# hrdkjain/GenIcoNet

Hardware: AMD Instinct MI355X
Metric: meshes/sec training throughput, ico2ico I5 batch=36 (higher is better)
Workload: dtype f32; 1 GPU; ico2ico AE training, I5, batch 36 per GPU (BASELINE configs[1]); per_gpu_batch=36, global_batch=36, subdivisions=5, parallelism=dp1

## Files before the change

geniconet_amd/_lib.py:

```python
import ctypes
import os
import types

import numpy as np
import torch

_HERE = os.path.dirname(os.path.abspath(__file__))
LIB_PATH = os.environ.get('ICN_LIB_PATH') or os.path.join(_HERE, 'libicn.so')

OP_CONV_FWD, OP_CONV_BWD_DATA, OP_CONV_BWD_WEIGHT = 0, 1, 2
CORNER_MODES = {'zeros': 0, 'average': 1}
ABI_VERSION = 9
LAP_MODES = {'mean-v': 0, 'v-mean': 1, 'sum-kv': 2, 'kv-sum': 3}

_c_float_p = ctypes.c_void_p
_i32p = ctypes.POINTER(ctypes.c_int32)
_f32p = ctypes.POINTER(ctypes.c_float)
_intp = ctypes.POINTER(ctypes.c_int)

RC, COUNT, PLAIN = 'rc', 'count', 'plain'

SIGNATURES = {
    'icn_abi_version': (ctypes.c_int, [], PLAIN),
    'icn_last_error': (ctypes.c_char_p, [], PLAIN),
    'icn_prepare_conv': (ctypes.c_int, [ctypes.c_int] * 3, RC),
    'icn_prepare_upsample': (ctypes.c_int, [ctypes.c_int] * 2, RC),
    'icn_conv_workspace_bytes': (ctypes.c_size_t, [ctypes.c_int] * 6, PLAIN),
    'icn_conv_fwd': (ctypes.c_int, [_c_float_p] * 4 + [ctypes.c_int] * 6 + [ctypes.c_void_p, ctypes.c_size_t, ctypes.c_void_p], RC),
    'icn_conv_bwd_data': (ctypes.c_int, [_c_float_p] * 3 + [ctypes.c_int] * 6 + [ctypes.c_void_p, ctypes.c_size_t, ctypes.c_void_p], RC),
    'icn_conv_bwd_weight': (ctypes.c_int, [_c_float_p] * 4 + [ctypes.c_int] * 6 + [ctypes.c_void_p, ctypes.c_size_t, ctypes.c_void_p], RC),
    'icn_conv_pair_supported': (ctypes.c_int, [ctypes.c_int] * 6, PLAIN),
    'icn_conv_pair_workspace_bytes': (ctypes.c_size_t, [ctypes.c_int] * 7, PLAIN),
    'icn_conv_pair_fwd': (ctypes.c_int, [_c_float_p] * 7 + [ctypes.c_int] * 7 + [ctypes.c_void_p, ctypes.c_size_t, ctypes.c_void_p], RC),
    'icn_conv_pair_bwd_data': (ctypes.c_int, [_c_float_p] * 5 + [ctypes.c_int] * 7 + [ctypes.c_void_p, ctypes.c_size_t, ctypes.c_void_p], RC),
    'icn_conv_pair_bwd_weight': (ctypes.c_int, [_c_float_p] * 7 + [ctypes.c_int] * 7 + [ctypes.c_void_p, ctypes.c_size_t, ctypes.c_void_p], RC),
    'icn_upconv_supported': (ctypes.c_int, [ctypes.c_int] * 5, PLAIN),
    'icn_upconv_workspace_bytes': (ctypes.c_size_t, [ctypes.c_int] * 5, PLAIN),
    'icn_upconv_fwd': (ctypes.c_int, [_c_float_p] * 7 + [ctypes.c_int] * 6 + [ctypes.c_void_p, ctypes.c_size_t, ctypes.c_void_p], RC),
    'icn_upconv_bwd_supported': (ctypes.c_int, [ctypes.c_int] * 6, PLAIN),
    'icn_upconv_bwd_workspace_bytes': (ctypes.c_size_t, [ctypes.c_int] * 5, PLAIN),
    'icn_upconv_bwd': (ctypes.c_int, [_c_float_p] * 10 + [ctypes.c_int] * 6 + [ctypes.c_void_p, ctypes.c_size_t, ctypes.c_void_p], RC),
    'icn_upconv_bwd_streams': (ctypes.c_int, [_c_float_p] * 10 + [ctypes.c_int] * 6 + [ctypes.c_void_p, ctypes.c_size_t, ctypes.c_void_p, ctypes.c_void_p], RC),
    'icn_upsample_fwd': (ctypes.c_int, [_c_float_p] * 2 + [ctypes.c_int] * 4 + [ctypes.c_void_p], RC),
    'icn_upsample_bwd': (ctypes.c_int, [_c_float_p] * 2 + [ctypes.c_int] * 4 + [ctypes.c_void_p], RC),
    'icn_bn_workspace_floats': (ctypes.c_size_t, [ctypes.c_int] * 2, PLAIN),
    'icn_bn_stats2': (ctypes.c_int, [_c_float_p, _c_float_p, ctypes.c_int, ctypes.c_int] + ([ctypes.c_float] * 2 + [_c_float_p] * 3) * 2 + [_c_float_p, ctypes.c_void_p], RC),
    'icn_bn_stats': (ctypes.c_int, [_c_float_p, ctypes.c_int, ctypes.c_int, ctypes.c_float, ctypes.c_float] + [_c_float_p] * 4 + [ctypes.c_void_p], RC),
    'icn_bn_relu_fwd': (ctypes.c_int, [_c_float_p] * 9 + [ctypes.c_int] * 2 + [ctypes.c_void_p], RC),
    'icn_bn_relu_bwd': (ctypes.c_int, [_c_float_p] * 13 + [ctypes.c_int] * 2 + [_c_float_p] * 4 + [ctypes.c_void_p], RC),
    'icn_head_workspace_floats': (ctypes.c_size_t, [ctypes.c_int] * 2, PLAIN),
    'icn_head_fwd': (ctypes.c_int, [_c_float_p] * 4 + [ctypes.c_int] * 3 + [ctypes.c_void_p], RC),
    'icn_head_bwd': (ctypes.c_int, [_c_float_p] * 8 + [ctypes.c_int] * 3 + [ctypes.c_void_p], RC),
    'icn_p2p_loss_workspace_floats': (ctypes.c_size_t, [ctypes.c_int] * 2, PLAIN),
    'icn_p2p_loss_fwd': (ctypes.c_int, [_c_float_p] * 2 + [ctypes.c_int] * 2 + [ctypes.c_float] * 3 + [ctypes.c_int] + [_c_float_p] * 2 + [ctypes.c_void_p], RC),
    'icn_p2p_loss_bwd_workspace_floats': (ctypes.c_size_t, [ctypes.c_int] * 2, PLAIN),
    'icn_p2p_loss_bwd': (ctypes.c_int, [_c_float_p] * 3 + [ctypes.c_int] * 2 + [ctypes.c_float] * 3 + [ctypes.c_int] + [_c_float_p] * 2 + [ctypes.c_void_p], RC),
    'icn_mesh_reg_workspace_floats': (ctypes.c_size_t, [ctypes.c_int] * 2, PLAIN),
    'icn_mesh_reg_fwd': (ctypes.c_int, [_c_float_p] + [ctypes.c_int] * 2 + [ctypes.c_float] * 4 + [_c_float_p] * 2 + [ctypes.c_void_p], RC),
    'icn_mesh_reg_bwd_workspace_floats': (ctypes.c_size_t, [ctypes.c_int] * 2, PLAIN),
    'icn_mesh_reg_bwd': (ctypes.c_int, [_c_float_p] * 2 + [ctypes.c_int] * 2 + [ctypes.c_float] * 4 + [_c_float_p] * 2 + [ctypes.c_void_p], RC),
    'icn_kld_workspace_floats': (ctypes.c_size_t, [ctypes.c_size_t], PLAIN),
    'icn_kld_fwd': (ctypes.c_int, [_c_float_p] * 2 + [ctypes.c_size_t] + [_c_float_p] * 2 + [ctypes.c_void_p], RC),
    'icn_kld_bwd': (ctypes.c_int, [_c_float_p] * 3 + [ctypes.c_size_t] + [_c_float_p] * 2 + [ctypes.c_void_p], RC),
    'icn_reparam_fwd': (ctypes.c_int, [_c_float_p] * 3 + [ctypes.c_size_t] + [_c_float_p] + [ctypes.c_void_p], RC),
    'icn_reparam_bwd': (ctypes.c_int, [_c_float_p] * 3 + [ctypes.c_size_t] + [_c_float_p] * 2 + [ctypes.c_void_p], RC),
    'icn_adam_step': (ctypes.c_int, [ctypes.c_int] + [ctypes.c_void_p] * 7 + [ctypes.c_double] * 4 + [ctypes.c_void_p], RC),
    'icn_adam_step_dev': (ctypes.c_int, [ctypes.c_int] + [ctypes.c_void_p] * 6 + [ctypes.c_double] * 4 + [ctypes.c_void_p], RC),
    'icn_table_stream_k': (ctypes.c_long, [ctypes.c_int] * 4 + [_i32p, ctypes.c_size_t], COUNT),
    'icn_table_tile_lists': (ctypes.c_long, [ctypes.c_int] * 7 + [_i32p, ctypes.c_size_t], COUNT),
    'icn_set_debug_flags': (ctypes.c_int, [ctypes.c_int], PLAIN),
    'icn_device_status': (ctypes.c_int, [ctypes.c_int], COUNT),
    'icn_get_arith': (ctypes.c_int, [], COUNT),
    'icn_set_arith': (ctypes.c_int, [ctypes.c_int], COUNT),
    'icn_build_flags': (ctypes.c_uint, [], PLAIN),
    'icn_host_selfcheck': (ctypes.c_long, [ctypes.c_int] * 2, COUNT),
    'icn_debug_trace': (ctypes.c_int, [ctypes.c_void_p, ctypes.c_size_t], RC),
    'icn_point_to_mesh': (ctypes.c_int, [_c_float_p] * 3 + [ctypes.c_int] * 4 + [_c_float_p] * 3 + [ctypes.c_void_p], RC),
    'icn_point_to_mesh_bwd_workspace_bytes': (ctypes.c_size_t, [ctypes.c_int] * 4, PLAIN),
    'icn_point_to_mesh_grid_workspace_bytes': (ctypes.c_size_t, [ctypes.c_int] * 4, PLAIN),
    'icn_point_to_mesh_grid': (ctypes.c_int, [_c_float_p] * 3 + [ctypes.c_int] * 4 + [_c_float_p] * 3 + [ctypes.c_void_p, ctypes.c_size_t, ctypes.c_void_p], RC),
    'icn_point_to_mesh_bwd': (ctypes.c_int, [_c_float_p] * 6 + [ctypes.c_int] * 4 + [_c_float_p] * 2 + [ctypes.c_void_p, ctypes.c_size_t, ctypes.c_void_p], RC),
    'icn_mesh_sample_workspace_bytes': (ctypes.c_size_t, [ctypes.c_int] * 4, PLAIN),
    'icn_mesh_sample_fwd': (ctypes.c_int, [_c_float_p] * 3 + [ctypes.c_int] * 4 + [_c_float_p] * 3 + [ctypes.c_void_p, ctypes.c_size_t, ctypes.c_void_p], RC),
    'icn_mesh_sample_bwd_workspace_bytes': (ctypes.c_size_t, [ctypes.c_int] * 4, PLAIN),
    'icn_mesh_sample_bwd': (ctypes.c_int, [_c_float_p] * 4 + [ctypes.c_int] * 4 + [_c_float_p] + [ctypes.c_void_p, ctypes.c_size_t, ctypes.c_void_p], RC),
    'icn_table_conv_fwd': (ctypes.c_long, [ctypes.c_int] * 3 + [_i32p, ctypes.c_size_t], COUNT),
    'icn_table_wgrad7': (ctypes.c_long, [ctypes.c_int] * 3 + [_i32p, ctypes.c_size_t, ctypes.POINTER(ctypes.c_uint16), ctypes.c_size_t, _intp], COUNT),
    'icn_table_conv_bwd': (ctypes.c_long, [ctypes.c_int] * 3 + [_i32p, ctypes.c_size_t, _intp], COUNT),
    'icn_table_upsample': (ctypes.c_long, [ctypes.c_int] * 3 + [_i32p, _f32p, ctypes.c_size_t, _intp], COUNT),
    'icn_table_upsample_pairs': (ctypes.c_long, [ctypes.c_int, _i32p, ctypes.c_size_t], COUNT),
    'icn_table_faces': (ctypes.c_long, [ctypes.c_int, _i32p, ctypes.c_size_t], COUNT),
    'icn_table_vertex_stencils': (ctypes.c_long, [ctypes.c_int, _i32p, ctypes.c_size_t], COUNT),
    'icn_table_upconv_bwd': (ctypes.c_long, [ctypes.c_int] * 2 + [_i32p, _f32p, ctypes.c_size_t, _intp], COUNT),
    'icn_table_upconv': (ctypes.c_long, [ctypes.c_int, ctypes.c_int, _i32p, ctypes.c_size_t, _f32p, ctypes.c_size_t, _intp], COUNT),
}

EXTENSION_HEADERS = {
    'icn_ext.h': {
        'icn_face_normal_agree_bwd_workspace_bytes': (ctypes.c_size_t, [ctypes.c_int] * 4, PLAIN),
        'icn_face_normal_agree_fwd': (ctypes.c_int, ([_c_float_p] * 3 + [ctypes.c_int] * 2) * 2 + [ctypes.c_int] * 3 + [_c_float_p, ctypes.c_void_p], RC),
        'icn_face_normal_agree_bwd': (ctypes.c_int, ([_c_float_p] * 3 + [ctypes.c_int] * 2) * 2 + [ctypes.c_int] * 3 + [_c_float_p] * 3
                                      + [ctypes.c_void_p, ctypes.c_size_t, ctypes.c_void_p], RC),
    },
    'icn_measure.h': {
        'icn_mesh_measure_workspace_bytes': (ctypes.c_size_t, [ctypes.c_int] * 3, PLAIN),
        'icn_mesh_measure_fwd': (ctypes.c_int, [_c_float_p] * 2 + [ctypes.c_int] * 3 + [_c_float_p] * 2 + [ctypes.c_void_p, ctypes.c_size_t, ctypes.c_void_p], RC),
        'icn_mesh_measure_bwd': (ctypes.c_int, [_c_float_p] * 6 + [ctypes.c_int] * 3 + [_c_float_p, ctypes.c_void_p], RC),
    },
    'icn_curvature.h': {
        'icn_mesh_cotlap_fwd': (ctypes.c_int, [_c_float_p] * 4 + [ctypes.c_int] * 3 + [_c_float_p] * 2 + [ctypes.c_void_p], RC),
        'icn_mesh_cotlap_bwd': (ctypes.c_int, [_c_float_p] * 6 + [ctypes.c_int] * 3 + [_c_float_p, ctypes.c_void_p], RC),
        'icn_mesh_willmore_workspace_bytes': (ctypes.c_size_t, [ctypes.c_int] * 3, PLAIN),
        'icn_mesh_willmore_fwd': (ctypes.c_int, [_c_float_p] * 4 + [ctypes.c_int] * 3 + [_c_float_p] * 3 + [ctypes.c_void_p, ctypes.c_size_t, ctypes.c_void_p], RC),
        'icn_mesh_willmore_bwd': (ctypes.c_int, [_c_float_p] * 7 + [ctypes.c_int] * 3 + [_c_float_p, ctypes.c_void_p, ctypes.c_size_t, ctypes.c_void_p], RC),
    },
    'icn_gauss.h': {
        'icn_mesh_angle_defect_fwd': (ctypes.c_int, [_c_float_p] * 4 + [ctypes.c_int] * 3 + [_c_float_p, ctypes.c_void_p], RC),
        'icn_mesh_angle_defect_bwd': (ctypes.c_int, [_c_float_p] * 5 + [ctypes.c_int] * 3 + [_c_float_p, ctypes.c_void_p], RC),
    },
    'icn_isect.h': {
        'icn_mesh_self_intersect': (ctypes.c_int, [_c_float_p] * 2 + [ctypes.c_int] * 3 + [_c_float_p, ctypes.c_void_p], RC),
    },
    'icn_sdf.h': {
        'icn_point_to_mesh_sign': (ctypes.c_int, [_c_float_p] * 8 + [ctypes.c_int] * 4 + [_c_float_p, ctypes.c_void_p], RC),
    },
    'icn_voxel.h': {
        'icn_mesh_voxelize': (ctypes.c_int, [_c_float_p] * 2 + [ctypes.c_int] * 3 + [ctypes.c_double] * 4 + [ctypes.c_int] * 3
                              + [ctypes.c_void_p, ctypes.c_void_p], RC),
    },
    'icn_raycast.h': {
        'icn_mesh_raycast': (ctypes.c_int, [_c_float_p] * 4 + [ctypes.c_int] * 4 + [_c_float_p] * 3 + [ctypes.c_void_p], RC),
        'icn_mesh_raycast_bwd_workspace_bytes': (ctypes.c_size_t, [ctypes.c_int] * 3, PLAIN),
        'icn_mesh_raycast_bwd': (ctypes.c_int, [_c_float_p] * 6 + [ctypes.c_int] * 4 + [_c_float_p] * 3
                                 + [ctypes.c_void_p, ctypes.c_size_t, ctypes.c_void_p], RC),
    },
    'icn_nn.h': {
        'icn_nearest_points': (ctypes.c_int, [_c_float_p] * 2 + [ctypes.c_int] * 3 + [_c_float_p] * 2 + [ctypes.c_void_p], RC),
        'icn_nearest_points_bwd_workspace_bytes': (ctypes.c_size_t, [ctypes.c_int] * 3, PLAIN),
        'icn_nearest_points_bwd': (ctypes.c_int, [_c_float_p] * 4 + [ctypes.c_int] * 3 + [_c_float_p] * 2
                                   + [ctypes.c_void_p, ctypes.c_size_t, ctypes.c_void_p], RC),
    },
}

LATER_HEADERS = {
    'icn_pairs.h': {
        'icn_sided_sums_workspace_bytes': (ctypes.c_size_t, [ctypes.c_int] * 4, PLAIN),
        'icn_sided_sums': (ctypes.c_int, [_c_float_p] * 2 + [ctypes.c_int] * 4 + [_c_float_p]
                           + [ctypes.c_void_p, ctypes.c_size_t, ctypes.c_void_p], RC),
    },
}
MATCH_HEADERS = {
    'icn_match.h': {
        'icn_match_clouds_workspace_bytes': (ctypes.c_size_t, [ctypes.c_int] * 4, PLAIN),
        'icn_match_clouds': (ctypes.c_int, [_c_float_p] * 2 + [ctypes.c_int] * 6 + [ctypes.c_void_p] * 4
                             + [ctypes.c_void_p, ctypes.c_size_t, ctypes.c_void_p], RC),
    },
}


class ProfileEntry(ctypes.Structure):
    _fields_ = [('kernel', ctypes.c_char_p), ('launches', ctypes.c_long), ('total_ms', ctypes.c_double),
                ('total_flops', ctypes.c_double)]


SIGNATURES['icn_profile_start'] = (ctypes.c_int, [ctypes.c_int], RC)
SIGNATURES['icn_profile_stop'] = (ctypes.c_int, [ctypes.POINTER(ProfileEntry), ctypes.c_int], COUNT)
SIGNATURES['icn_profile_select'] = (ctypes.c_int, [ctypes.c_char_p], RC)

_lib = _api = None


def _raises(name, reply, last_error):
    def errcheck(result, func, args):
        if result < 0 or (result and reply == RC):
            raise RuntimeError('%s failed: %s' % (name, last_error().decode()))
        return result
    return errcheck


def lib():
    global _lib, _api
    if _lib is None:
        if not os.path.exists(LIB_PATH):
            raise RuntimeError(
                'geniconet_amd: %s is missing -- the HIP extension is the product and has no fallback. '
                'Build it with `python -c "import __graft_entry__ as g; g.build()"` '
                '(or `make -C geniconet_amd/csrc`).' % LIB_PATH)
        handle = ctypes.CDLL(LIB_PATH)
        checked = types.SimpleNamespace()
        for name, (res, args, reply) in [item for table in (SIGNATURES, *EXTENSION_HEADERS.values(), *LATER_HEADERS.values(), *MATCH_HEADERS.values()) for item in table.items()]:
            fn = getattr(handle, name)
            fn.restype, fn.argtypes = res, args
            fn = handle[name]
            fn.restype, fn.argtypes = res, args
            if reply != PLAIN:
                fn.errcheck = _raises(name, reply, handle.icn_last_error)
            setattr(checked, name, fn)
        if handle.icn_abi_version() != ABI_VERSION:
            raise RuntimeError('geniconet_amd: libicn.so ABI %d != binding ABI %d; rebuild'
                               % (handle.icn_abi_version(), ABI_VERSION))
        refuse_pricing_build(handle.icn_build_flags(), LIB_PATH)
        _lib, _api = handle, checked
    return _lib


def api():
    return _api or (lib() and _api)


def stream():
    return torch.cuda.current_stream().cuda_stream


def workspace(n, device, dtype=torch.uint8):
    return torch.empty(max(int(n), 1), dtype=dtype, device=device)


def refuse_pricing_build(flags, path, allow=None):
    exp = flags & 0xffff
    allow = os.environ.get('ICN_ALLOW_EXP') == '1' if allow is None else allow
    if exp and not allow:
        raise RuntimeError('geniconet_amd: %s is a pricing build (ICN_EXP=%d: a feature of the convolution kernel is compiled out, '
                           'its RESULTS ARE WRONG by design); set ICN_ALLOW_EXP=1 to time it' % (path, exp))


def build_info():
    f = api().icn_build_flags()
    return dict(path=LIB_PATH, overridden=bool(os.environ.get('ICN_LIB_PATH')), exp=f & 0xffff, conv_waves_default=(f >> 16) & 0xff,
                chain_prio=(f >> 24) & 0xf)


ARITH_MODES = {'f32': 0, 'bf16x3': 1}


def get_arith():
    return {0: 'f32', 1: 'bf16x3'}[api().icn_get_arith()]


def set_arith(mode):
    return {0: 'f32', 1: 'bf16x3'}[api().icn_set_arith(ARITH_MODES[mode])]


def source_files():
    import glob
    headers = [os.path.join(os.path.dirname(_HERE), 'include', h) for h in ('icn.h', *EXTENSION_HEADERS, *LATER_HEADERS, *MATCH_HEADERS)]
    return sorted([f for pattern in ('*.hip', '*.h', '*.cpp') for f in glob.glob(os.path.join(_HERE, 'csrc', pattern))] + headers)


def source_sha256():
    import hashlib
    h = hashlib.sha256()
    for f in source_files():
        h.update(os.path.basename(f).encode() + b'\0')
        h.update(open(f, 'rb').read())
    return h.hexdigest()


def check(rc, what):
    if rc != 0:
        raise RuntimeError('%s failed: %s' % (what, lib().icn_last_error().decode()))


STATUS_BITS = {1: "a stream-K workgroup of k_conv_dma_sk never received a partner's partial tile (the tile was set to NaN)"}


def device_status(device=None, clear=True, synchronize=True):
    with torch.cuda.device(device):
        if synchronize:
            torch.cuda.synchronize()
        return api().icn_device_status(1 if clear else 0)


def raise_on_device_status(device=None, synchronize=True):
    v = device_status(device, synchronize=synchronize)
    if v:
        raise RuntimeError('libicn: asynchronous kernel failure on %s: %s' % (
            device if device is not None else 'the current device',
            '; '.join(msg for bit, msg in STATUS_BITS.items() if v & bit) or 'status 0x%x' % v))


def corner_code(corner_mode):
    try:
        return CORNER_MODES[corner_mode]
    except KeyError:
        raise ValueError("corner_mode must be 'zeros' or 'average', got %r" % (corner_mode,))


def _table(name, ints, outs, sizes=None):
    fn = getattr(api(), name)

    def call(bufs):
        args, k = list(ints), -1
        for o in outs:
            if o == 'cap':
                args.append(bufs[k].size if bufs else 0)
            elif isinstance(o, type):
                k += 1
                args.append(bufs[k].ctypes.data_as(fn.argtypes[len(args)]) if bufs else None)
            else:
                args.append(o)
        return fn(*args)
    n = call(None)
    dtypes = [o for o in outs if isinstance(o, type)]
    bufs = [np.empty(m, dtype=d) for d, m in zip(dtypes, sizes(n) if sizes else [n] * len(dtypes))]
    call(bufs)
    return bufs


def table_conv_fwd(r_in, stride, corner_mode):
    out, = _table('icn_table_conv_fwd', (r_in, stride, corner_code(corner_mode)), (np.int32, 'cap'))
    return out.reshape(7, -1)


def table_wgrad7(r_in, stride, corner_mode):
    meta = (ctypes.c_int * 2)()
    rows, pos = _table('icn_table_wgrad7', (r_in, stride, corner_code(corner_mode)), (np.int32, 'cap', np.uint16, 'cap', meta),
                       lambda n: (n, meta[1] * 16 * 8))
    return (rows.reshape(meta[1], meta[0]), pos.reshape(meta[1], 16, 8)) if rows.size else None


def table_conv_bwd(r_in, stride, corner_mode):
    w = ctypes.c_int(0)
    out, = _table('icn_table_conv_bwd', (r_in, stride, corner_code(corner_mode)), (np.int32, 'cap', ctypes.byref(w)))
    return out.reshape(7, w.value, -1)


def table_upsample(r_in, corner_mode, transpose=False):
    w = ctypes.c_int(0)
    idx, coef = _table('icn_table_upsample', (r_in, corner_code(corner_mode), int(transpose)),
                       (np.int32, np.float32, 'cap', ctypes.byref(w)))
    return idx.reshape(-1, w.value), coef.reshape(-1, w.value)


def table_faces(r):
    return _table('icn_table_faces', (r,), (np.int32, 'cap'))[0].reshape(-1, 3)


def table_vertex_stencils(r):
    return _table('icn_table_vertex_stencils', (r,), (np.int32, 'cap'))[0].reshape(-1, 6, 3)


def table_upsample_pairs(r_in):
    return _table('icn_table_upsample_pairs', (r_in,), (np.int32, 'cap'))[0].reshape(2, -1)


def table_upconv(r_in, corner_mode):
    meta = (ctypes.c_int * 7)()
    ints, floats = _table('icn_table_upconv', (r_in, corner_code(corner_mode)), (np.int32, 'cap', np.float32, 'cap', meta),
                          lambda n: (n, meta[6]))
    Pf, Pc, n_slots, E, nseg, NV, _ = list(meta)
    o = 0
    seg = ints[o:o + 3 * nseg].reshape(nseg, 3); o += 3 * nseg
    pix = ints[o:o + Pf]; o += Pf
    code = ints[o:o + NV * Pf].reshape(NV, Pf); o += NV * Pf
    slot_idx = ints[o:o + n_slots * E].reshape(n_slots, E)
    return dict(Pf=Pf, Pc=Pc, seg=seg, pix=pix, code=code, alpha=floats[:NV * 7].reshape(NV, 7), slot_idx=slot_idx,
                slot_coef=floats[NV * 7:].reshape(n_slots, E))


def table_upconv_bwd(r_in, corner_mode):
    w = ctypes.c_int(0)
    idx, coef = _table('icn_table_upconv_bwd', (r_in, corner_code(corner_mode)), (np.int32, np.float32, 'cap', ctypes.byref(w)))
    return idx.reshape(-1, w.value), coef.reshape(-1, w.value)


def table_stream_k(ntiles, grid, nk, ku=1):
    return _table('icn_table_stream_k', (ntiles, grid, nk, ku), (np.int32, 'cap'))[0].reshape(-1, 4)


def table_tile_lists(r_in, B, bm, ntn, grid, corner_mode='average'):
    out, = _table('icn_table_tile_lists', (r_in, 2, corner_code(corner_mode), B, bm, ntn, grid), (np.int32, 'cap'))
    return out[:grid + 1], out[grid + 1:]


def profile_start(max_launches=4096, only=None):
    api().icn_profile_select(only.encode() if only else None)
    api().icn_profile_start(max_launches)


def profile_stop():
    buf = (ProfileEntry * 48)()
    n = api().icn_profile_stop(buf, 48)
    return [dict(kernel=buf[i].kernel.decode(), launches=buf[i].launches, total_ms=buf[i].total_ms,
                 total_flops=buf[i].total_flops) for i in range(n)]
```

geniconet_amd/csrc/icn_api.cpp:

```cpp
#include <hip/hip_runtime.h>

#include <algorithm>
#include <cmath>
#include <cstdio>
#include <cstdlib>
#include <cstring>
#include <map>
#include <mutex>
#include <stdexcept>
#include <string>
#include <tuple>
#include <vector>

#include "../../include/icn_ext.h"
#include "../../include/icn_curvature.h"
#include "../../include/icn_gauss.h"
#include "../../include/icn_isect.h"
#include "../../include/icn_sdf.h"
#include "../../include/icn_voxel.h"
#include "../../include/icn_raycast.h"
#include "../../include/icn_nn.h"
#include "../../include/icn_pairs.h"
#include "../../include/icn_match.h"
#include "../../include/icn_measure.h"
#include "icn_geometry.h"
#include "icn_launch.h"
#include "icn_streamk.h"

namespace {

thread_local std::string g_err;

int fail(const std::string& msg) {
    g_err = msg;
    return -1;
}

#define ICN_HIP(expr)                                                                       \
    do {                                                                                    \
        hipError_t e_ = (expr);                                                             \
        if (e_ != hipSuccess) throw std::runtime_error(std::string(#expr) + ": " + hipGetErrorString(e_)); \
    } while (0)

template <typename R, typename F>
R returns(F&& body) {
    try {
        return body();
    } catch (const std::exception& e) {
        return (R)fail(e.what());
    }
}
template <typename R, typename F>
R returns_or_zero(F&& body) {
    try {
        return body();
    } catch (const std::exception&) {
        return 0;
    }
}
template <typename F>
int guarded(F&& body) {
    return returns<int>([&] { body(); return 0; });
}
template <typename F>
int launched(F&& body) {
    return returns<int>([&] { body(); ICN_HIP(hipGetLastError()); return 0; });
}

template <typename T>
long copy_out(T* dst, size_t cap, const std::vector<T>& v) {
    if (dst) std::memcpy(dst, v.data(), std::min(cap, v.size()) * sizeof(T));
    return (long)v.size();
}

thread_local bool g_dry_run = false;
thread_local size_t g_dry_elems = 0;

template <typename T>
T* upload(const std::vector<T>& v) {
    T* d = nullptr;
    if (v.empty()) return d;
    if (g_dry_run) {
        g_dry_elems += v.size();
        return d;
    }
    ICN_HIP(hipMalloc(reinterpret_cast<void**>(&d), v.size() * sizeof(T)));
    ICN_HIP(hipMemcpy(d, v.data(), v.size() * sizeof(T), hipMemcpyHostToDevice));
    return d;
}

struct DevDma {
    int32_t* code = nullptr;
    int32_t* slots = nullptr;
    int n_slots = 0, E = 1;
};
DevDma upload_dma(const std::vector<int32_t>& idx, int E, int P) {
    icn::DmaTable h;
    icn::build_dma_table(idx, E, P, h);
    DevDma d;
    d.code = upload(h.code);
    d.slots = upload(h.slots);
    d.n_slots = h.n_slots;
    d.E = E;
    return d;
}
struct ConvTables {
    int Pin = 0, Pout = 0, n_in = 0, n_out = 0, E = 1;
    int32_t* fwd = nullptr;
    int32_t* bwd = nullptr;
    int32_t* bwd1 = nullptr;
    int nv = 0, nvp = 0;
    int32_t* vidx = nullptr;
    int32_t* vorder = nullptr;
    uint32_t* vmask32 = nullptr;
    int32_t* vq = nullptr;
    int32_t* perm = nullptr;
    int32_t* bwd_perm = nullptr;
    uint32_t* mask32 = nullptr;
    std::vector<uint32_t> mask32_h;
    int key = 0;
    DevDma d_fwd, d_bwd, d_bwd1, d_virt, d_bwdp;
    int32_t* w7_rows = nullptr;
    uint16_t* w7_pos = nullptr;
    int w7_U = 0;
};
struct UpTables {
    int Pc = 0, Pf = 0, Wf = 0, Wb = 0;
    int32_t *idx_f = nullptr, *idx_b = nullptr;
    float *coef_f = nullptr, *coef_b = nullptr;
};

struct UpconvDev {
    int Pc = 0, Pf = 0, n_slots = 0, E = 1, nseg = 0;
    int seg_cnt[icn::UPCONV_MAX_SEG] = {}, seg_off[icn::UPCONV_MAX_SEG] = {};
    uint32_t seg_mask[icn::UPCONV_MAX_SEG] = {};
    int32_t *pix = nullptr, *code = nullptr, *slot_idx = nullptr;
    float *alpha = nullptr, *slot_coef = nullptr;
};

struct EllSplitDev {
    int W = 0, n_ovf = 0, W_ovf = 0;
    int32_t *idx = nullptr, *ovf_rows = nullptr, *ovf_idx = nullptr;
    float *coef = nullptr, *ovf_coef = nullptr;
};
EllSplitDev upload_ell_split(const icn::Ell& e, int W_main) {
    EllSplitDev d;
    const int W = e.width;
    d.W = W_main;
    d.W_ovf = std::max(W - W_main, 0);
    std::vector<int32_t> idx((size_t)e.rows * W_main, icn::IDX_ZERO), ovf_rows, ovf_idx;
    std::vector<float> coef((size_t)e.rows * W_main, 0.f), ovf_coef;
    for (int r = 0; r < e.rows; ++r) {
        for (int k = 0; k < std::min(W, W_main); ++k) {
            idx[(size_t)r * W_main + k] = e.idx[(size_t)r * W + k];
            coef[(size_t)r * W_main + k] = e.coef[(size_t)r * W + k];
        }
        if (W > W_main && e.idx[(size_t)r * W + W_main] != icn::IDX_ZERO) {
            ovf_rows.push_back(r);
            for (int k = W_main; k < W; ++k) {
                ovf_idx.push_back(e.idx[(size_t)r * W + k]);
                ovf_coef.push_back(e.coef[(size_t)r * W + k]);
            }
        }
    }
    d.n_ovf = (int)ovf_rows.size();
    d.idx = upload(idx);
    d.coef = upload(coef);
    d.ovf_rows = upload(ovf_rows);
    d.ovf_idx = upload(ovf_idx);
    d.ovf_coef = upload(ovf_coef);
    return d;
}

struct PatchHost { std::vector<int32_t> prow; std::vector<uint16_t> plocal; int npatch = 0, umax = 0, gridW = 0; };
bool build_patches(const std::vector<int32_t>& idx, int width_in, int width, int H, int W, int ph, int pw, PatchHost& out) {
    out = PatchHost{};
    if (H % ph != 0 || W % pw != 0 || (long)H * W * width_in != (long)idx.size()) return false;
    const int pr_n = H / ph, pc_n = W / pw;
    out.npatch = pr_n * pc_n;
    out.gridW = W;
    out.plocal.assign((size_t)H * W * width, 0xFFFFu);
    std::vector<std::vector<int32_t>> lists(out.npatch);
    for (int p = 0; p < out.npatch; ++p) {
        std::vector<int32_t>& u = lists[p];
        for (int i = 0; i < ph; ++i)
            for (int j = 0; j < pw; ++j) {
                const size_t r = (size_t)((p / pc_n) * ph + i) * W + (p % pc_n) * pw + j;
                for (int k = 0; k < width; ++k) {
                    const int32_t v = idx[r * width_in + k];
                    if (v >= 0) u.push_back(v);
                }
            }
        std::sort(u.begin(), u.end());
        u.erase(std::unique(u.begin(), u.end()), u.end());
        out.umax = std::max(out.umax, (int)u.size());
    }
    out.umax = (out.umax + 31) / 32 * 32;
    if (out.umax == 0 || out.umax >= 0xFFFF) return false;
    out.prow.assign((size_t)out.npatch * out.umax, -1);
    for (int p = 0; p < out.npatch; ++p) {
        const std::vector<int32_t>& u = lists[p];
        std::copy(u.begin(), u.end(), out.prow.begin() + (size_t)p * out.umax);
        for (int i = 0; i < ph; ++i)
            for (int j = 0; j < pw; ++j) {
                const size_t r = (size_t)((p / pc_n) * ph + i) * W + (p % pc_n) * pw + j;
                for (int k = 0; k < width; ++k) {
                    const int32_t v = idx[r * width_in + k];
                    if (v >= 0) out.plocal[r * width + k] = (uint16_t)(std::lower_bound(u.begin(), u.end(), v) - u.begin());
                }
            }
    }
    return true;
}
struct PatchDev { int32_t* prow = nullptr; uint16_t* plocal = nullptr; int npatch = 0, umax = 0, gridW = 0; };
PatchDev upload_patches(const PatchHost& h) {
    PatchDev d;
    if (getenv("ICN_VERBOSE")) fprintf(stderr, "icn: patch table: %d patches, %d rows per list, grid width %d\n", h.npatch, h.umax, h.gridW);
    d.prow = upload(h.prow);
    d.plocal = upload(h.plocal);
    d.npatch = h.npatch; d.umax = h.umax; d.gridW = h.gridW;
    return d;
}

struct UpconvBwdDev {
    int Pc = 0, Pf = 0;
    PatchDev sc_patch, ga_patch;
    EllSplitDev gather, scatter;
    int32_t* iota = nullptr;
    int32_t* px_srcs = nullptr;
    int32_t* px_cls = nullptr;
    float* cls_coef = nullptr;
    int n_cls = 0;
};

std::mutex g_mu;
std::map<std::tuple<int, int, int>, UpconvDev> g_upconv;
std::map<std::tuple<int, int, int>, UpconvBwdDev> g_upconv_bwd;
std::map<std::tuple<int, int, int, int>, ConvTables> g_conv;
std::map<std::tuple<int, int, int>, UpTables> g_up;

static int wgrad7_union_rows(int stride) {
    if (stride != 1) return 112;
    static const int u1 = [] {
        const char* e = getenv("ICN_W7_U");
        return e ? atoi(e) : 64;
    }();
    if (u1 != 56 && u1 != 64)
        throw std::invalid_argument("icn: ICN_W7_U must be 56 or 64 (the instantiations of k_wgrad7 at stride 1), got " + std::to_string(u1));
    return u1;
}

ConvTables make_conv_tables(int r_in, int stride, int mode) {
    ConvTables t;
    t.n_in = 1 << r_in;
    t.n_out = t.n_in / stride;
    t.Pin = icn::pixels(r_in);
    t.Pout = 10 * t.n_out * t.n_out;
    std::vector<int32_t> fwd, bwd, perm;
    std::vector<uint8_t> mask;
    icn::build_conv_fwd(r_in, stride, mode, fwd);
    t.E = icn::build_conv_bwd(r_in, stride, mode, bwd);
    t.fwd = upload(fwd);
    t.bwd = upload(bwd);
    t.d_fwd = upload_dma(fwd, 1, t.Pout);
    t.d_bwd = upload_dma(bwd, t.E, t.Pin);
    {
        icn::DmaTable h;
        icn::build_dma_table(fwd, 1, t.Pout, h);
        icn::Wg7Table w7;
        if (icn::build_wgrad7(h, t.Pout, wgrad7_union_rows(stride), w7)) {
            t.w7_rows = upload(w7.urow);
            t.w7_pos = upload(w7.upos);
            t.w7_U = w7.U;
        }
    }
    std::vector<int32_t> primary;
    icn::VirtualRows vr;
    icn::split_conv_bwd(r_in, stride, bwd, t.E, primary, vr);
    t.bwd1 = upload(primary);
    t.d_bwd1 = upload_dma(primary, 1, t.Pin);
    t.nv = vr.nv;
    if (vr.nv > 0) {
        std::vector<int32_t> order, vidx_o;
        std::vector<uint8_t> vmask;
        icn::build_virtual_order(vr, t.nvp, order, vidx_o, vmask);
        t.vidx = upload(vidx_o);
        t.vorder = upload(order);
        t.vmask32 = upload(std::vector<uint32_t>(vmask.begin(), vmask.end()));
        t.d_virt = upload_dma(vidx_o, 1, t.nvp);
        t.vq = upload(vr.vq);
    }
    if (stride == 2) {
        icn::build_bwd_row_order(r_in, stride, bwd, t.E, perm, mask);
        t.perm = upload(perm);
        t.mask32_h.assign(mask.begin(), mask.end());
        t.mask32 = upload(t.mask32_h);
        t.key = 1 + ((r_in << 8) | (stride << 4) | mode);
        std::vector<int32_t> bwd_p(bwd.size());
        for (int te = 0; te < icn::NTAPS * t.E; ++te)
            for (int k = 0; k < t.Pin; ++k) bwd_p[(size_t)te * t.Pin + k] = bwd[(size_t)te * t.Pin + perm[k]];
        t.bwd_perm = upload(bwd_p);
        t.d_bwdp = upload_dma(bwd_p, t.E, t.Pin);
    }
    return t;
}
const ConvTables& conv_tables(int r_in, int stride, int mode) {
    int dev = 0;
    ICN_HIP(hipGetDevice(&dev));
    std::lock_guard<std::mutex> lk(g_mu);
    auto key = std::make_tuple(dev, r_in, stride, mode);
    auto it = g_conv.find(key);
    if (it != g_conv.end()) return it->second;
    return g_conv.emplace(key, make_conv_tables(r_in, stride, mode)).first->second;
}

std::map<std::pair<int, int>, int32_t*> g_vf;

const int32_t* vertex_faces(int r) {
    int dev = 0;
    ICN_HIP(hipGetDevice(&dev));
    std::lock_guard<std::mutex> lk(g_mu);
    auto key = std::make_pair(dev, r);
    auto it = g_vf.find(key);
    if (it != g_vf.end()) return it->second;
    std::vector<int32_t> vf;
    icn::build_vertex_faces(r, vf);
// ... 1195 lines not shown
            throw std::invalid_argument("icn_mesh_voxelize: bad sizes");
        icn::launch_mesh_voxelize(vertices, faces, B, V, F, origin_x, origin_y, origin_z, spacing, n0, n1, n2, occupancy, s);
    });
}

namespace {
bool raycast_rays_ok(int B, int R, int V) { return mesh_sizes_ok(B, R, V, 1) && R <= 0x7fffffff / 3; }
}

int icn_mesh_raycast(const float* origins, const float* directions, const float* vertices, const int32_t* faces, int B, int R, int V, int F,
                     float* depth, int32_t* face, int32_t* count, void* stream) {
    hipStream_t s = static_cast<hipStream_t>(stream);
    return launched([&] {
        if (!origins || !directions || !vertices || !faces || !depth || !face || !count)
            throw std::invalid_argument("icn_mesh_raycast: null pointer");
        check_measure_sizes("icn_mesh_raycast", B, V, F);
        if (!raycast_rays_ok(B, R, V)) throw std::invalid_argument("icn_mesh_raycast: bad sizes");
        icn::launch_mesh_raycast(origins, directions, vertices, faces, B, R, V, F, depth, face, count, s);
    });
}

size_t icn_mesh_raycast_bwd_workspace_bytes(int B, int R, int V) {
    return raycast_rays_ok(B, R, V) ? icn::vertex_records_bytes((size_t)B * R) : 0;
}

int icn_mesh_raycast_bwd(const float* origins, const float* directions, const float* vertices, const int32_t* faces, const int32_t* face,
                         const float* ddepth, int B, int R, int V, int F, float* dorigins, float* ddirections, float* dvertices, void* ws,
                         size_t ws_bytes, void* stream) {
    hipStream_t s = static_cast<hipStream_t>(stream);
    return guarded([&] {
        if (!origins || !directions || !vertices || !faces || !face || !ddepth) throw std::invalid_argument("icn_mesh_raycast_bwd: null pointer");
        check_measure_sizes("icn_mesh_raycast_bwd", B, V, F);
        if (!raycast_rays_ok(B, R, V)) throw std::invalid_argument("icn_mesh_raycast_bwd: bad sizes");
        if (!dorigins && !ddirections && !dvertices) return;
        if (dvertices) check_workspace("icn_mesh_raycast_bwd", ws, ws_bytes, icn::vertex_records_bytes((size_t)B * R));
        icn::launch_mesh_raycast_bwd(origins, directions, vertices, faces, face, ddepth, B, R, V, F, dorigins, ddirections, dvertices, ws, s);
        ICN_HIP(hipGetLastError());
    });
}

namespace {
bool nearest_sizes_ok(int B, int N, int M) { return mesh_sizes_ok(B, N, M, 1) && N <= 0x7fffffff / 3 && M <= 0x7fffffff / 3; }
}

int icn_nearest_points(const float* points, const float* targets, int B, int N, int M, float* dist, int32_t* idx, void* stream) {
    hipStream_t s = static_cast<hipStream_t>(stream);
    return launched([&] {
        if (!points || !targets || !dist || !idx) throw std::invalid_argument("icn_nearest_points: null pointer");
        if (!nearest_sizes_ok(B, N, M)) throw std::invalid_argument("icn_nearest_points: bad sizes");
        icn::launch_nearest_points(points, targets, B, N, M, dist, idx, s);
    });
}

size_t icn_nearest_points_bwd_workspace_bytes(int B, int N, int M) {
    return nearest_sizes_ok(B, N, M) ? icn::vertex_records_bytes((size_t)B * N) : 0;
}

int icn_nearest_points_bwd(const float* points, const float* targets, const int32_t* idx, const float* ddist, int B, int N, int M,
                           float* dpoints, float* dtargets, void* ws, size_t ws_bytes, void* stream) {
    hipStream_t s = static_cast<hipStream_t>(stream);
    return guarded([&] {
        if (!points || !targets || !idx || !ddist) throw std::invalid_argument("icn_nearest_points_bwd: null pointer");
        if (!nearest_sizes_ok(B, N, M)) throw std::invalid_argument("icn_nearest_points_bwd: bad sizes");
        if (!dpoints && !dtargets) return;
        if (dtargets) check_workspace("icn_nearest_points_bwd", ws, ws_bytes, icn::vertex_records_bytes((size_t)B * N));
        icn::launch_nearest_points_bwd(points, targets, idx, ddist, B, N, M, dpoints, dtargets, ws, s);
        ICN_HIP(hipGetLastError());
    });
}

namespace {
bool sided_sums_sizes_ok(int G, int R, int N, int M) { return nearest_sizes_ok(G, N, M) && R >= 1 && R <= 65535; }
}

size_t icn_sided_sums_workspace_bytes(int G, int R, int N, int M) {
    return sided_sums_sizes_ok(G, R, N, M) ? icn::sided_sums_workspace_bytes(G, R, N) : 0;
}

int icn_sided_sums(const float* queries, const float* targets, int G, int R, int N, int M, double* sums, void* ws, size_t ws_bytes,
                   void* stream) {
    hipStream_t s = static_cast<hipStream_t>(stream);
    return launched([&] {
        if (!queries || !targets || !sums) throw std::invalid_argument("icn_sided_sums: null pointer");
        if (!sided_sums_sizes_ok(G, R, N, M)) throw std::invalid_argument("icn_sided_sums: bad sizes");
        check_workspace("icn_sided_sums", ws, ws_bytes, icn::sided_sums_workspace_bytes(G, R, N));
        icn::launch_sided_sums(queries, targets, G, R, N, M, sums, ws, s);
    });
}

namespace {
bool match_sizes_ok(int G, int R, int N, int paired, int phases, int max_rounds) {
    return nearest_sizes_ok(G, N, N) && R >= 1 && R <= 65535 && icn::match_clouds_fits(N) && (paired == 0 || (paired == 1 && G == R)) &&
           phases >= 1 && phases <= 26 && max_rounds >= 1;
}
}

size_t icn_match_clouds_workspace_bytes(int G, int R, int N, int paired) {
    return match_sizes_ok(G, R, N, paired, 1, 1) ? icn::match_clouds_workspace_bytes(G, R, N, paired) : 0;
}

int icn_match_clouds(const float* queries, const float* targets, int G, int R, int N, int paired, int phases, int max_rounds,
                     int* match, double* prices, double* cost, int* rounds, void* ws, size_t ws_bytes, void* stream) {
    hipStream_t s = static_cast<hipStream_t>(stream);
    return launched([&] {
        if (!queries || !targets || !cost || !rounds) throw std::invalid_argument("icn_match_clouds: null pointer");
        if (!match_sizes_ok(G, R, N, paired, phases, max_rounds)) throw std::invalid_argument("icn_match_clouds: bad sizes");
        check_workspace("icn_match_clouds", ws, ws_bytes, icn::match_clouds_workspace_bytes(G, R, N, paired));
        icn::launch_match_clouds(queries, targets, G, R, N, paired, phases, max_rounds, match, prices, cost, rounds, ws, s);
    });
}

int icn_adam_step(int count, float* const* params, const float* const* grads, float* const* exp_avg, float* const* exp_avg_sq,
                  const size_t* numel, const float* step_size, const float* bc2_sqrt, double beta1, double beta2, double eps,
                  double weight_decay, void* stream) {
    hipStream_t s = static_cast<hipStream_t>(stream);
    return guarded([&] {
        check_adam("icn_adam_step", count, params, grads, exp_avg, exp_avg_sq, numel, count > 0 && (!step_size || !bc2_sqrt), beta1, beta2, eps);
        if (count == 0) return;
        icn::launch_adam(count, params, grads, exp_avg, exp_avg_sq, numel, step_size, bc2_sqrt, beta1, beta2, eps, weight_decay, s);
        ICN_HIP(hipGetLastError());
    });
}

int icn_adam_step_dev(int count, float* const* params, const float* const* grads, float* const* exp_avg, float* const* exp_avg_sq,
                      const size_t* numel, const float* scalars_dev, double beta1, double beta2, double eps, double weight_decay,
                      void* stream) {
    hipStream_t s = static_cast<hipStream_t>(stream);
    return guarded([&] {
        check_adam("icn_adam_step_dev", count, params, grads, exp_avg, exp_avg_sq, numel, !scalars_dev, beta1, beta2, eps);
        if (count == 0) return;
        std::vector<float> same(count, 0.f);
        icn::launch_adam(count, params, grads, exp_avg, exp_avg_sq, numel, same.data(), same.data(), beta1, beta2, eps, weight_decay, s,
                         scalars_dev);
        ICN_HIP(hipGetLastError());
    });
}

long icn_table_stream_k(int ntiles, int grid, int nk, int ku, int32_t* out, size_t cap) {
    return returns<long>([&] {
        if (ntiles < 1 || grid < 8 || grid % 8 != 0 || nk < 1 || ku < 1)
            throw std::invalid_argument("icn_table_stream_k: grid must be a positive multiple of 8, nk and ku positive");
        size_t n = 0;
        std::vector<int> tables(2 * (grid / 8 + 1));
        const int occ = grid / 256;
        icn::sk_tables(ntiles, grid, nk, ku, occ, grid % 256 == 0 ? icn::sk_speed_factors(occ) : nullptr, tables.data());
        for (int b = 0; b < grid; ++b) {
            icn::SkWalk w{};
            w.init(b, grid, ntiles, nk, ku, tables.data());
            int tile, k0, k1;
            while (w.next(tile, k0, k1)) {
                if (out && n + 4 <= cap) { out[n] = b; out[n + 1] = tile; out[n + 2] = k0; out[n + 3] = k1; }
                n += 4;
            }
        }
        return (long)n;
    });
}

long icn_table_tile_lists(int r_in, int stride, int corner_mode, int B, int bm, int ntn, int grid, int32_t* out, size_t cap) {
    return returns<long>([&] {
        if (r_in < 1 || r_in > 8 || stride != 2 || B < 1 || (bm != 64 && bm != 128) || ntn < 1 || grid < 8 || grid % 256 != 0)
            throw std::invalid_argument("icn_table_tile_lists: stride-2 tables, bm 64 / 128, grid a multiple of 256");
        std::vector<int32_t> bwd, perm;
        std::vector<uint8_t> mask;
        const int E = icn::build_conv_bwd(r_in, stride, corner_mode, bwd);
        icn::build_bwd_row_order(r_in, stride, bwd, E, perm, mask);
        const std::vector<uint32_t> m32(mask.begin(), mask.end());
        const int Pd = icn::pixels(r_in), M = B * Pd, ntiles = ((M + bm - 1) / bm) * ntn;
        std::vector<int> h;
        icn::build_tile_lists(m32.data(), M, Pd, bm, ntn, ntiles, grid, grid / 256, h);
        return copy_out(out, cap, h);
    });
}

int icn_set_debug_flags(int flags) { return icn::set_debug_flags(flags); }

int icn_get_arith(void) {
    return returns<int>([&] { return icn::arith_mode(); });
}
int icn_set_arith(int mode) {
    return returns<int>([&] { return icn::set_arith_mode(mode); });
}
unsigned icn_build_flags(void) { return icn::build_flags(); }

int icn_debug_trace(void* device_buffer, size_t n_u64) {
    icn::set_trace_buffer(device_buffer, n_u64);
    return 0;
}

long icn_host_selfcheck(int r, int corner_mode) {
    return returns<long>([&] {
        if (r < 0 || r > 7 || (corner_mode != 0 && corner_mode != 1)) throw std::invalid_argument("icn_host_selfcheck: r in [0, 7], corner_mode 0 / 1");
        g_dry_run = true;
        g_dry_elems = 0;
        struct Reset { ~Reset() { g_dry_run = false; } } reset;
        (void)make_conv_tables(r, 1, corner_mode);
        if (r >= 1) (void)make_conv_tables(r, 2, corner_mode);
        (void)make_up_tables(r, corner_mode);
        (void)make_upconv_tables(r, corner_mode);
        (void)make_upconv_bwd_tables(r, corner_mode);
        std::vector<int32_t> vf;
        icn::build_vertex_faces(r, vf);
        (void)upload(vf);
        (void)table_counts(r, 1);
        if (r >= 1) (void)table_counts(r, 2);
        (void)upconv_slots(r);
        const int chans[] = {64, 128, 256, 512};
        size_t plan = 0;
        for (int B : {1, 3, 36})
            for (int ci : chans)
                for (int co : chans) {
                    for (int stride = 1; stride <= (r >= 1 ? 2 : 1); ++stride) {
                        for (int op = 0; op < 3; ++op) plan += conv_ws_bytes(op, B, ci, co, 0, r, stride) != 0;
                        if (pair_supported(B, ci, co, co, r, stride))
                            for (int op = 0; op < 3; ++op) plan += conv_ws_bytes(op, B, ci, co, co, r, stride) != 0;
                        const int n_out = (1 << r) / stride, M = B * 10 * n_out * n_out;
                        plan += (size_t)icn::wgrad_splits(M, ci, co, 0);
                    }
                    plan += icn_upconv_workspace_bytes(B, ci, co, co, r) != 0;
                    plan += icn_upconv_bwd_workspace_bytes(B, ci, co, co, r) != 0;
                }
        return (long)(g_dry_elems + plan);
    });
}

int icn_device_status(int clear) {
    return returns<int>([&] { return icn::device_status(clear); });
}

size_t icn_bn_workspace_floats(int M, int C) { return (M < 1 || C < 1) ? 0 : (size_t)icn::bn_chunks(M) * 4 * C * 2; }

int icn_bn_stats(const float* x, int M, int C, float eps, float momentum, float* running_mean, float* running_var, float* stat,
                 float* ws, void* stream) {
    hipStream_t s = static_cast<hipStream_t>(stream);
    return launched([&] {
        if (!x || !stat || !ws || M < 1) throw std::invalid_argument("icn_bn_stats: bad arguments");
        if (!icn::bn_supported(C)) throw std::invalid_argument("icn_bn_stats: unsupported channel count");
        icn::launch_bn_stats(x, M, C, eps, momentum, running_mean, running_var, stat, ws, s);
    });
}

int icn_bn_stats2(const float* a, const float* b, int M, int C, float eps_a, float momentum_a, float* running_mean_a,
                  float* running_var_a, float* stat_a, float eps_b, float momentum_b, float* running_mean_b, float* running_var_b,
                  float* stat_b, float* ws, void* stream) {
    hipStream_t s = static_cast<hipStream_t>(stream);
    return launched([&] {
        if (!a || !b || !stat_a || !stat_b || !ws || M < 1) throw std::invalid_argument("icn_bn_stats2: bad arguments");
        if ((running_mean_a == nullptr) != (running_var_a == nullptr) || (running_mean_b == nullptr) != (running_var_b == nullptr))
            throw std::invalid_argument("icn_bn_stats2: running mean and variance go together");
        if (!icn::bn_supported(C)) throw std::invalid_argument("icn_bn_stats2: unsupported channel count");
        icn::launch_bn_stats2(a, b, M, C, eps_a, momentum_a, running_mean_a, running_var_a, stat_a, eps_b, momentum_b, running_mean_b,
                              running_var_b, stat_b, ws, s);
    });
}

int icn_bn_relu_fwd(const float* a, const float* b, const float* stat_a, const float* stat_b, const float* gamma_a,
                    const float* beta_a, const float* gamma_b, const float* beta_b, float* y, int M, int C, void* stream) {
    hipStream_t s = static_cast<hipStream_t>(stream);
    return launched([&] {
        if (!a || !stat_a || !gamma_a || !beta_a || !y || M < 1) throw std::invalid_argument("icn_bn_relu_fwd: bad arguments");
        if (b && (!stat_b || !gamma_b || !beta_b)) throw std::invalid_argument("icn_bn_relu_fwd: second input needs its stats");
        if (!icn::bn_supported(C)) throw std::invalid_argument("icn_bn_relu_fwd: unsupported channel count");
        icn::launch_bn_relu_fwd(a, b, stat_a, stat_b, gamma_a, beta_a, gamma_b, beta_b, y, M, C, s);
    });
}

int icn_bn_relu_bwd(const float* dy, const float* a, const float* b, const float* stat_a, const float* stat_b, const float* gamma_a,
                    const float* beta_a, const float* gamma_b, const float* beta_b, float* da, float* db, float* sums, float* ws, int M,
                    int C, float* dbeta_a, float* dgamma_a, float* dbeta_b, float* dgamma_b, void* stream) {
    hipStream_t s = static_cast<hipStream_t>(stream);
    return launched([&] {
        if (!dy || !a || !stat_a || !gamma_a || !beta_a || !da || !sums || !ws || M < 1)
            throw std::invalid_argument("icn_bn_relu_bwd: bad arguments");
        if (b && (!stat_b || !gamma_b || !beta_b || !db)) throw std::invalid_argument("icn_bn_relu_bwd: second input needs its buffers");
        if (!icn::bn_supported(C)) throw std::invalid_argument("icn_bn_relu_bwd: unsupported channel count");
        icn::launch_bn_relu_bwd(dy, a, b, stat_a, stat_b, gamma_a, beta_a, gamma_b, beta_b, da, db, sums, ws, M, C, dbeta_a, dgamma_a,
                                dbeta_b, dgamma_b, s);
    });
}

size_t icn_head_workspace_floats(int M, int Cin) {
    return (M < 1 || Cin < 1) ? 0 : (size_t)icn::head_chunks(M) * 4 * (Cin + 4) * (icn::head_sums_in_double(M) ? 2 : 1);
}

int icn_head_fwd(const float* x, const float* w, const float* bias, float* y, int M, int Cin, int Cout, void* stream) {
    hipStream_t s = static_cast<hipStream_t>(stream);
    return launched([&] {
        if (!x || !w || !bias || !y || M < 1) throw std::invalid_argument("icn_head_fwd: bad arguments");
        if (!icn::head_supported(Cin, Cout)) throw std::invalid_argument("icn_head_fwd: unsupported channel counts");
        icn::launch_head_fwd(x, w, bias, y, M, Cin, Cout, s);
    });
}

int icn_head_bwd(const float* dy, const float* y, const float* x, const float* w, float* dx, float* dw, float* db, float* ws,
                 int M, int Cin, int Cout, void* stream) {
    hipStream_t s = static_cast<hipStream_t>(stream);
    return launched([&] {
        if (!dy || !y || !x || !w || !dw || !db || !ws || M < 1) throw std::invalid_argument("icn_head_bwd: bad arguments");
        if (!icn::head_supported(Cin, Cout)) throw std::invalid_argument("icn_head_bwd: unsupported channel counts");
        icn::launch_head_bwd(dy, y, x, w, dx, dw, db, ws, M, Cin, Cout, s);
    });
}

long icn_table_conv_fwd(int r_in, int stride, int corner_mode, int32_t* out, size_t cap) {
    return returns<long>([&] {
        std::vector<int32_t> v;
        icn::build_conv_fwd(r_in, stride, corner_mode, v);
        return copy_out(out, cap, v);
    });
}

long icn_table_wgrad7(int r_in, int stride, int corner_mode, int32_t* rows, size_t cap_rows, uint16_t* pos, size_t cap_pos, int* meta) {
    return returns<long>([&] {
        std::vector<int32_t> fwd;
        icn::build_conv_fwd(r_in, stride, corner_mode, fwd);
        const int P = (int)(fwd.size() / icn::NTAPS);
        icn::DmaTable h;
        icn::build_dma_table(fwd, 1, P, h);
        icn::Wg7Table w7;
        if (!icn::build_wgrad7(h, P, wgrad7_union_rows(stride), w7)) {
            if (meta) meta[0] = meta[1] = 0;
            return 0L;
        }
        if (meta) { meta[0] = w7.U; meta[1] = w7.npatch; }
        copy_out(pos, cap_pos, w7.upos);
        return copy_out(rows, cap_rows, w7.urow);
    });
}

long icn_table_conv_bwd(int r_in, int stride, int corner_mode, int32_t* out, size_t cap, int* width) {
    return returns<long>([&] {
        std::vector<int32_t> v;
        const int E = icn::build_conv_bwd(r_in, stride, corner_mode, v);
        if (width) *width = E;
        return copy_out(out, cap, v);
    });
}

long icn_table_upsample(int r_in, int corner_mode, int transpose, int32_t* idx, float* coef, size_t cap, int* width) {
    return returns<long>([&] {
        icn::Ell f, b;
        icn::build_upsample(r_in, corner_mode, f, b);
        const icn::Ell& e = transpose ? b : f;
        if (width) *width = e.width;
        copy_out(coef, cap, e.coef);
        return copy_out(idx, cap, e.idx);
    });
}

long icn_table_upsample_pairs(int r_in, int32_t* out, size_t cap) {
    return returns<long>([&] {
        std::vector<int32_t> v;
        icn::build_upsample_pairs(r_in, v);
        return copy_out(out, cap, v);
    });
}

long icn_table_upconv(int r_in, int corner_mode, int32_t* ints, size_t cap_ints, float* floats, size_t cap_floats, int* meta) {
    return returns<long>([&] {
        icn::UpconvTable t;
        icn::build_upconv_fwd(r_in, corner_mode, t);
        std::vector<int32_t> iv;
        for (int sg = 0; sg < t.nseg; ++sg) {
            iv.push_back(t.seg_cnt[sg]);
            iv.push_back(t.seg_off[sg]);
            iv.push_back((int32_t)t.seg_mask[sg]);
        }
        iv.insert(iv.end(), t.pix.begin(), t.pix.end());
        iv.insert(iv.end(), t.code.begin(), t.code.end());
        iv.insert(iv.end(), t.slot_idx.begin(), t.slot_idx.end());
        std::vector<float> fv(t.alpha);
        fv.insert(fv.end(), t.slot_coef.begin(), t.slot_coef.end());
        if (meta) {
            meta[0] = t.Pf; meta[1] = t.Pc; meta[2] = t.n_slots; meta[3] = t.E; meta[4] = t.nseg; meta[5] = icn::UPCONV_TAPS;
            meta[6] = (int)fv.size();
        }
        copy_out(floats, cap_floats, fv);
        return copy_out(ints, cap_ints, iv);
    });
}

long icn_table_upconv_bwd(int r_in, int corner_mode, int32_t* idx, float* coef, size_t cap, int* width) {
    return returns<long>([&] {
        icn::Ell e;
        icn::build_upconv_bwd(r_in, corner_mode, e);
        if (width) *width = e.width;
        copy_out(coef, cap, e.coef);
        return copy_out(idx, cap, e.idx);
    });
}

long icn_table_faces(int r, int32_t* out, size_t cap) {
    return returns<long>([&] {
        std::vector<int32_t> v;
        icn::build_faces(r, v);
        return copy_out(out, cap, v);
    });
}

long icn_table_vertex_stencils(int r, int32_t* out, size_t cap) {
    return returns<long>([&] {
        std::vector<int32_t> v;
        icn::build_vertex_stencils(r, v);
        return copy_out(out, cap, v);
    });
}

}
```

geniconet_amd/csrc/icn_bn.hip:

```cpp
#include <hip/hip_runtime.h>
#include <stdint.h>

#include <algorithm>

#include "icn_launch.h"

#ifndef ICN_CHAIN_PRIO
#define ICN_CHAIN_PRIO 0
#endif
#if ICN_CHAIN_PRIO > 0
#define ICN_CHAIN_SETPRIO() __builtin_amdgcn_s_setprio(ICN_CHAIN_PRIO)
#else
#define ICN_CHAIN_SETPRIO() ((void)0)
#endif

namespace icn {

using f32x4 = __attribute__((ext_vector_type(4))) float;
__device__ __forceinline__ f32x4 ldv(const float* p) { return *reinterpret_cast<const f32x4*>(p); }
__device__ __forceinline__ void stv(float* p, f32x4 v) { *reinterpret_cast<f32x4*>(p) = v; }
__device__ __forceinline__ f32x4 relu4(f32x4 v) { return f32x4{fmaxf(v[0], 0.f), fmaxf(v[1], 0.f), fmaxf(v[2], 0.f), fmaxf(v[3], 0.f)}; }

#ifndef ICN_BN_MAX_CHUNKS
#define ICN_BN_MAX_CHUNKS 512
#endif
constexpr int BN_MAX_CHUNKS = ICN_BN_MAX_CHUNKS;
static_assert(BN_MAX_CHUNKS >= 1 && BN_MAX_CHUNKS <= 65536, "ICN_BN_MAX_CHUNKS");

using f64x4 = __attribute__((ext_vector_type(4))) double;
__device__ __forceinline__ f64x4 to_d(f32x4 v) { return f64x4{(double)v[0], (double)v[1], (double)v[2], (double)v[3]}; }

template <int DUAL>
__device__ __forceinline__ f32x4 bn_pre4(f32x4 a, f32x4 mean_a, f32x4 scale_a, f32x4 beta_a, f32x4 b, f32x4 mean_b, f32x4 scale_b,
                                         f32x4 beta_b) {
    f32x4 v = (a - mean_a) * scale_a + beta_a;
    if (DUAL) v += (b - mean_b) * scale_b + beta_b;
    return v;
}

#ifndef ICN_BN_UN
#define ICN_BN_UN 4
#endif
#ifndef ICN_BN_UN_BWD
#define ICN_BN_UN_BWD 2
#endif
#ifndef ICN_BN_WAVES
#define ICN_BN_WAVES 1
#endif
static_assert(ICN_BN_WAVES >= 1 && ICN_BN_WAVES <= 8, "ICN_BN_WAVES: minimum workgroups per CU of k_bn_partial's launch bounds");
template <int MODE>
__global__ __launch_bounds__(256, ICN_BN_WAVES) void k_bn_partial(const float* __restrict__ p0, const float* __restrict__ p2,
                                                     const float* __restrict__ p3, const float* __restrict__ stat_a,
                                                     const float* __restrict__ stat_b, const float* __restrict__ ga,
                                                     const float* __restrict__ ba, const float* __restrict__ gb,
                                                     const float* __restrict__ bb, double* __restrict__ partial, int M, int C,
                                                     int rows_per_chunk) {
    ICN_CHAIN_SETPRIO();
    constexpr int NS = MODE == 3 ? 4 : (MODE == 2 ? 3 : 2);
    __shared__ f64x4 red[NS][256];
    const int c4n = C / 4, stripes = 256 / c4n;
    const int cq = threadIdx.x % c4n, stripe = threadIdx.x / c4n, c = cq * 4;
    const int r0 = blockIdx.x * rows_per_chunk, r1 = min(M, r0 + rows_per_chunk);
    constexpr int UN = (MODE == 1 || MODE == 2) ? ICN_BN_UN_BWD : ICN_BN_UN;
    static_assert(UN == 1 || UN == 2 || UN == 4, "ICN_BN_UN / ICN_BN_UN_BWD: the accumulator combine below is written for 1, 2 or 4 rows per iteration");
    f64x4 s[UN][NS];
#pragma unroll
    for (int u = 0; u < UN; ++u)
#pragma unroll
        for (int k = 0; k < NS; ++k) s[u][k] = f64x4{0.0, 0.0, 0.0, 0.0};
    f32x4 mean_a{}, inv_a{}, mean_b{}, inv_b{}, sc_a{}, sc_b{}, be_a{}, be_b{};
    if (MODE == 1 || MODE == 2) { mean_a = ldv(stat_a + c); inv_a = ldv(stat_a + C + c); sc_a = inv_a * ldv(ga + c); be_a = ldv(ba + c); }
    if (MODE == 2) { mean_b = ldv(stat_b + c); inv_b = ldv(stat_b + C + c); sc_b = inv_b * ldv(gb + c); be_b = ldv(bb + c); }
    f32x4 shift{}, shift_b{};
    if (MODE == 0 || MODE == 3) shift = ldv(p0 + c);
    if (MODE == 3) shift_b = ldv(p2 + c);
    if (stripe < stripes) {
        for (int r = r0 + stripe; r < r1; r += UN * stripes) {
            f32x4 x0[UN], x2[UN], x3[UN];
#pragma unroll
            for (int u = 0; u < UN; ++u) {
                const int ru = r + u * stripes;
                const size_t o = (size_t)min(ru, r1 - 1) * C + c;
                x0[u] = ldv(p0 + o);
                if (MODE >= 1) x2[u] = ldv(p2 + o);
                if (MODE == 2) x3[u] = ldv(p3 + o);
            }
#pragma unroll
            for (int u = 0; u < UN; ++u) {
                if (r + u * stripes >= r1) continue;
                if (MODE == 0 || MODE == 3) {
                    const f64x4 x = to_d(x0[u] - shift);
                    s[u][0] += x;
                    s[u][1] += x * x;
                    if (MODE == 3) {
                        const f64x4 xb = to_d(x2[u] - shift_b);
                        s[u][NS - 2] += xb;
                        s[u][NS - 1] += xb * xb;
                    }
                } else {
                    const f32x4 dy = x0[u], av = x2[u];
                    f32x4 bv{};
                    if (MODE == 2) bv = x3[u];
                    const f32x4 v = bn_pre4<MODE == 2>(av, mean_a, sc_a, be_a, bv, mean_b, sc_b, be_b);
                    f32x4 g;
#pragma unroll
                    for (int j = 0; j < 4; ++j) g[j] = v[j] > 0.f ? dy[j] : 0.f;
                    s[u][0] += to_d(g);
                    s[u][1] += to_d(g) * to_d((av - mean_a) * inv_a);
                    if (MODE == 2) s[u][2] += to_d(g) * to_d((bv - mean_b) * inv_b);
                }
            }
        }
    }
#pragma unroll
    for (int k = 0; k < NS; ++k) {
        if (UN == 4) s[0][k] = (s[0][k] + s[1][k]) + (s[2][k] + s[3][k]);
        else if (UN == 2) s[0][k] = s[0][k] + s[1][k];
    }
#pragma unroll
    for (int k = 0; k < NS; ++k) red[k][threadIdx.x] = s[0][k];
    __syncthreads();
    if (stripe == 0) {
#pragma unroll
        for (int k = 0; k < NS; ++k) {
            f64x4 t = red[k][cq];
            for (int q = 1; q < stripes; ++q) t += red[k][q * c4n + cq];
            *reinterpret_cast<f64x4*>(partial + ((size_t)blockIdx.x * NS + k) * C + c) = t;
        }
    }
}

template <int NQ>
__device__ __forceinline__ void chunk_sums(const double* __restrict__ partial, int chunks, int NS, int k0, int C, int c, int slice,
                                           double (*red)[16], double* out) {
    double s[NQ][4];
#pragma unroll
    for (int q = 0; q < NQ; ++q)
#pragma unroll
        for (int e = 0; e < 4; ++e) s[q][e] = 0.0;
    if (c < C) {
        const double* p = partial + (size_t)k0 * C + c;
        const size_t st = (size_t)NS * C;
        for (int j = slice; j < chunks; j += 128) {
            double v[NQ][8];
#pragma unroll
            for (int u = 0; u < 8; ++u)
#pragma unroll
                for (int q = 0; q < NQ; ++q) v[q][u] = j + 16 * u < chunks ? p[(size_t)(j + 16 * u) * st + (size_t)q * C] : 0.0;
#pragma unroll
            for (int q = 0; q < NQ; ++q)
#pragma unroll
                for (int u = 0; u < 8; ++u) s[q][u & 3] += v[q][u];
        }
    }
#pragma unroll
    for (int q = 0; q < NQ; ++q) {
        red[slice][threadIdx.x % 16] = (s[q][0] + s[q][1]) + (s[q][2] + s[q][3]);
        __syncthreads();
        double t = 0.0;
        if (slice == 0)
            for (int r = 0; r < 16; ++r) t += red[r][threadIdx.x % 16];
        __syncthreads();
        out[q] = t;
    }
}

__global__ __launch_bounds__(256) void k_bn_finalize_fwd(const float* __restrict__ x, const double* __restrict__ partial, int chunks,
                                                          int M, int C, float eps, float momentum,
                                                          float* __restrict__ running_mean, float* __restrict__ running_var,
                                                          float* __restrict__ stat) {
    __shared__ double red[16][16];
    const int c = blockIdx.x * 16 + threadIdx.x % 16, slice = threadIdx.x / 16;
    double sums[2];
    chunk_sums<2>(partial, chunks, 2, 0, C, c, slice, red, sums);
    const double s = sums[0], s2 = sums[1];
    if (slice != 0 || c >= C) return;
    const double ms = s / M;
    const double mean = (double)x[c] + ms;
    double var = s2 / M - ms * ms;
    if (var < 0.0) var = 0.0;
    stat[c] = (float)mean;
    stat[C + c] = (float)(1.0 / sqrt(var + (double)eps));
    if (running_mean) {
        const double unbiased = M > 1 ? var * M / (M - 1) : var;
        running_mean[c] = (1.f - momentum) * running_mean[c] + momentum * (float)mean;
        running_var[c] = (1.f - momentum) * running_var[c] + momentum * (float)unbiased;
    }
}

struct BnFin { const float* x; float eps, momentum; float* running_mean; float* running_var; float* stat; };
__global__ __launch_bounds__(256) void k_bn_finalize_fwd2(const BnFin fa, const BnFin fb, const double* __restrict__ partial, int chunks,
                                                           int M, int C) {
    __shared__ double red[16][16];
    const BnFin f = blockIdx.y ? fb : fa;
    const int c = blockIdx.x * 16 + threadIdx.x % 16, slice = threadIdx.x / 16;
    double sums[2];
    chunk_sums<2>(partial, chunks, 4, 2 * blockIdx.y, C, c, slice, red, sums);
    if (slice != 0 || c >= C) return;
    const double ms = sums[0] / M;
    const double mean = (double)f.x[c] + ms;
    double var = sums[1] / M - ms * ms;
    if (var < 0.0) var = 0.0;
    f.stat[c] = (float)mean;
    f.stat[C + c] = (float)(1.0 / sqrt(var + (double)f.eps));
    if (f.running_mean) {
        const double unbiased = M > 1 ? var * M / (M - 1) : var;
        f.running_mean[c] = (1.f - f.momentum) * f.running_mean[c] + f.momentum * (float)mean;
        f.running_var[c] = (1.f - f.momentum) * f.running_var[c] + f.momentum * (float)unbiased;
    }
}

struct BnGradOut { float* dbeta_a; float* dbeta_b; float* dgamma_a; float* dgamma_b; };
__global__ __launch_bounds__(256) void k_bn_finalize_bwd(const double* __restrict__ partial, int chunks, int C, int NS,
                                                          float* __restrict__ sums, const BnGradOut out) {
    __shared__ double red[16][16];
    const int c = blockIdx.x * 16 + threadIdx.x % 16, slice = threadIdx.x / 16, k = blockIdx.y;
    double s;
    chunk_sums<1>(partial, chunks, NS, k, C, c, slice, red, &s);
    if (slice == 0 && c < C) {
        const float v = (float)s;
        sums[k * C + c] = v;
        if (k == 0) {
            if (out.dbeta_a) out.dbeta_a[c] = v;
            if (out.dbeta_b) out.dbeta_b[c] = v;
        } else if (k == 1) {
            if (out.dgamma_a) out.dgamma_a[c] = v;
        } else if (out.dgamma_b) {
            out.dgamma_b[c] = v;
        }
    }
}

#ifndef ICN_BN_APPLY_UNR
#define ICN_BN_APPLY_UNR 1
#endif
constexpr int APPLY_UNR = ICN_BN_APPLY_UNR;
static_assert(APPLY_UNR >= 1 && APPLY_UNR <= 8, "ICN_BN_APPLY_UNR: elements per thread and iteration of the apply passes");

template <int DUAL>
__global__ void k_bn_relu_fwd(const float* __restrict__ a, const float* __restrict__ b, const float* __restrict__ stat_a,
                              const float* __restrict__ stat_b, const float* __restrict__ ga, const float* __restrict__ ba,
                              const float* __restrict__ gb, const float* __restrict__ bb, float* __restrict__ y, size_t total4,
                              int C) {
    ICN_CHAIN_SETPRIO();
    const size_t T = (size_t)gridDim.x * blockDim.x;
    for (size_t i0 = (size_t)blockIdx.x * blockDim.x + threadIdx.x; i0 < total4; i0 += APPLY_UNR * T) {
        f32x4 av[APPLY_UNR], bv[APPLY_UNR];
#pragma unroll
        for (int u = 0; u < APPLY_UNR; ++u) {
            const size_t i = i0 + u * T < total4 ? i0 + u * T : i0;
            av[u] = ldv(a + i * 4);
            if (DUAL) bv[u] = ldv(b + i * 4);
        }
#pragma unroll
        for (int u = 0; u < APPLY_UNR; ++u) {
            const size_t i = i0 + u * T;
            if (i >= total4) break;
            const int c = (int)((i * 4) % C);
            f32x4 bu{}, mb{}, sb{}, bbv{};
            if (DUAL) { bu = bv[u]; mb = ldv(stat_b + c); sb = ldv(stat_b + C + c) * ldv(gb + c); bbv = ldv(bb + c); }
            const f32x4 v = bn_pre4<DUAL>(av[u], ldv(stat_a + c), ldv(stat_a + C + c) * ldv(ga + c), ldv(ba + c), bu, mb, sb, bbv);
            stv(y + i * 4, relu4(v));
        }
    }
}

template <int DUAL>
__global__ void k_bn_relu_bwd(const float* __restrict__ dy, const float* __restrict__ a, const float* __restrict__ b,
                              const float* __restrict__ stat_a, const float* __restrict__ stat_b, const float* __restrict__ ga,
                              const float* __restrict__ ba, const float* __restrict__ gb, const float* __restrict__ bb,
                              const float* __restrict__ sums, float* __restrict__ da, float* __restrict__ db, size_t total4, int C,
                              float inv_m) {
    ICN_CHAIN_SETPRIO();
    const size_t T = (size_t)gridDim.x * blockDim.x;
    for (size_t i0 = (size_t)blockIdx.x * blockDim.x + threadIdx.x; i0 < total4; i0 += APPLY_UNR * T) {
        f32x4 dv[APPLY_UNR], avv[APPLY_UNR], bvv[APPLY_UNR];
#pragma unroll
        for (int u = 0; u < APPLY_UNR; ++u) {
            const size_t i = i0 + u * T < total4 ? i0 + u * T : i0;
            dv[u] = ldv(dy + i * 4);
            avv[u] = ldv(a + i * 4);
            if (DUAL) bvv[u] = ldv(b + i * 4);
        }
#pragma unroll
        for (int u = 0; u < APPLY_UNR; ++u) {
            const size_t i = i0 + u * T;
            if (i >= total4) break;
            const int c = (int)((i * 4) % C);
            const f32x4 d = dv[u], av = avv[u];
            const f32x4 mean_a = ldv(stat_a + c), inv_a = ldv(stat_a + C + c), gam_a = ldv(ga + c);
            f32x4 bv{}, mean_b{}, inv_b{}, gam_b{}, be_b{};
            if (DUAL) { bv = bvv[u]; mean_b = ldv(stat_b + c); inv_b = ldv(stat_b + C + c); gam_b = ldv(gb + c); be_b = ldv(bb + c); }
            const f32x4 v = bn_pre4<DUAL>(av, mean_a, inv_a * gam_a, ldv(ba + c), bv, mean_b, inv_b * gam_b, be_b);
            f32x4 g;
#pragma unroll
            for (int j = 0; j < 4; ++j) g[j] = v[j] > 0.f ? d[j] : 0.f;
            const f32x4 sg = ldv(sums + c) * inv_m;
            {
                const f32x4 xh = (av - mean_a) * inv_a;
                stv(da + i * 4, gam_a * inv_a * (g - sg - xh * (ldv(sums + C + c) * inv_m)));
            }
            if (DUAL) {
                const f32x4 xh = (bv - mean_b) * inv_b;
                stv(db + i * 4, gam_b * inv_b * (g - sg - xh * (ldv(sums + 2 * C + c) * inv_m)));
            }
        }
    }
}

bool bn_supported(int C) { return C >= 4 && C <= 1024 && C % 4 == 0 && 256 % (C / 4) == 0; }
int bn_chunks(int M) { return std::min(BN_MAX_CHUNKS, (M + 63) / 64); }

static int stream_blocks(size_t total4) { return (int)std::min((size_t)8192, (total4 + 256 * APPLY_UNR - 1) / (256 * APPLY_UNR)); }

void launch_bn_stats(const float* x, int M, int C, float eps, float momentum, float* running_mean, float* running_var, float* stat,
                     float* ws, hipStream_t s) {
    const int chunks = bn_chunks(M), rows = (M + chunks - 1) / chunks;
    hipLaunchKernelGGL(k_bn_partial<0>, dim3(chunks), dim3(256), 0, s, x, nullptr, nullptr, nullptr, nullptr, nullptr, nullptr, nullptr,
                       nullptr, reinterpret_cast<double*>(ws), M, C, rows);
    hipLaunchKernelGGL(k_bn_finalize_fwd, dim3((C + 15) / 16), dim3(256), 0, s, x, reinterpret_cast<const double*>(ws), chunks, M, C, eps, momentum, running_mean,
                       running_var, stat);
}

void launch_bn_stats2(const float* a, const float* b, int M, int C, float eps_a, float mom_a, float* rm_a, float* rv_a, float* stat_a,
                      float eps_b, float mom_b, float* rm_b, float* rv_b, float* stat_b, float* ws, hipStream_t s) {
    const int chunks = bn_chunks(M), rows = (M + chunks - 1) / chunks;
    hipLaunchKernelGGL(k_bn_partial<3>, dim3(chunks), dim3(256), 0, s, a, b, nullptr, nullptr, nullptr, nullptr, nullptr, nullptr,
                       nullptr, reinterpret_cast<double*>(ws), M, C, rows);
    hipLaunchKernelGGL(k_bn_finalize_fwd2, dim3((C + 15) / 16, 2), dim3(256), 0, s, BnFin{a, eps_a, mom_a, rm_a, rv_a, stat_a},
                       BnFin{b, eps_b, mom_b, rm_b, rv_b, stat_b}, reinterpret_cast<const double*>(ws), chunks, M, C);
}

void launch_bn_relu_fwd(const float* a, const float* b, const float* stat_a, const float* stat_b, const float* ga, const float* ba,
                        const float* gb, const float* bb, float* y, int M, int C, hipStream_t s) {
    const size_t total4 = (size_t)M * C / 4;
    if (b) hipLaunchKernelGGL(k_bn_relu_fwd<1>, dim3(stream_blocks(total4)), dim3(256), 0, s, a, b, stat_a, stat_b, ga, ba, gb, bb, y, total4, C);
    else hipLaunchKernelGGL(k_bn_relu_fwd<0>, dim3(stream_blocks(total4)), dim3(256), 0, s, a, b, stat_a, stat_b, ga, ba, gb, bb, y, total4, C);
}

void launch_bn_relu_bwd(const float* dy, const float* a, const float* b, const float* stat_a, const float* stat_b, const float* ga,
                        const float* ba, const float* gb, const float* bb, float* da, float* db, float* sums, float* ws, int M, int C,
                        float* dbeta_a, float* dgamma_a, float* dbeta_b, float* dgamma_b, hipStream_t s) {
    const int chunks = bn_chunks(M), rows = (M + chunks - 1) / chunks;
    const int NS = b ? 3 : 2;
    double* wsd = reinterpret_cast<double*>(ws);
    if (b) hipLaunchKernelGGL(k_bn_partial<2>, dim3(chunks), dim3(256), 0, s, dy, a, b, stat_a, stat_b, ga, ba, gb, bb, wsd, M, C, rows);
    else hipLaunchKernelGGL(k_bn_partial<1>, dim3(chunks), dim3(256), 0, s, dy, a, b, stat_a, stat_b, ga, ba, gb, bb, wsd, M, C, rows);
    hipLaunchKernelGGL(k_bn_finalize_bwd, dim3((C + 15) / 16, NS), dim3(256), 0, s, wsd, chunks, C, NS, sums,
                       BnGradOut{dbeta_a, b ? dbeta_b : nullptr, dgamma_a, b ? dgamma_b : nullptr});
    const size_t total4 = (size_t)M * C / 4;
    if (b) hipLaunchKernelGGL(k_bn_relu_bwd<1>, dim3(stream_blocks(total4)), dim3(256), 0, s, dy, a, b, stat_a, stat_b, ga, ba, gb, bb, sums, da, db, total4, C, 1.f / M);
    else hipLaunchKernelGGL(k_bn_relu_bwd<0>, dim3(stream_blocks(total4)), dim3(256), 0, s, dy, a, b, stat_a, stat_b, ga, ba, gb, bb, sums, da, db, total4, C, 1.f / M);
}

}

namespace icn {

constexpr int HEAD_MAX_OUT = 4;

template <int LPR>
__global__ __launch_bounds__(256) void k_head_fwd(const float* __restrict__ x, const float* __restrict__ w,
                                                   const float* __restrict__ bias, float* __restrict__ y, int M, int Cout) {
    constexpr int Cin = LPR * 4, RPB = 256 / LPR;
    const int sub = threadIdx.x % LPR, rloc = threadIdx.x / LPR;
    f32x4 wv[HEAD_MAX_OUT];
#pragma unroll
    for (int o = 0; o < HEAD_MAX_OUT; ++o) wv[o] = o < Cout ? ldv(w + o * Cin + 4 * sub) : f32x4{0.f, 0.f, 0.f, 0.f};
    for (int r = blockIdx.x * RPB + rloc; r < M; r += gridDim.x * RPB) {
        const f32x4 xv = ldv(x + (size_t)r * Cin + 4 * sub);
        float acc[HEAD_MAX_OUT];
#pragma unroll
        for (int o = 0; o < HEAD_MAX_OUT; ++o) acc[o] = xv[0] * wv[o][0] + xv[1] * wv[o][1] + xv[2] * wv[o][2] + xv[3] * wv[o][3];
#pragma unroll
        for (int d = LPR / 2; d >= 1; d >>= 1)
#pragma unroll
            for (int o = 0; o < HEAD_MAX_OUT; ++o) acc[o] += __shfl_xor(acc[o], d, 64);
        if (sub < Cout) {
            float v = acc[0];
#pragma unroll
            for (int o = 1; o < HEAD_MAX_OUT; ++o) v = sub == o ? acc[o] : v;
            y[(size_t)r * Cout + sub] = tanhf(v + bias[sub]);
        }
    }
}

constexpr int HEAD_F64_ROWS = 1024;
template <typename ACC> struct HeadAcc;
template <> struct HeadAcc<float> { using v4 = f32x4; static __device__ __forceinline__ v4 of(f32x4 v) { return v; } };
template <> struct HeadAcc<double> { using v4 = f64x4; static __device__ __forceinline__ v4 of(f32x4 v) { return to_d(v); } };

template <int LPR, typename ACC>
__global__ __launch_bounds__(256) void k_head_bwd(const float* __restrict__ dy, const float* __restrict__ y,
                                                   const float* __restrict__ x, const float* __restrict__ w,
                                                   float* __restrict__ dx, ACC* __restrict__ partial, int M, int Cout,
                                                   int rows_per_block) {
    using acc4 = typename HeadAcc<ACC>::v4;
    constexpr int Cin = LPR * 4, RPB = 256 / LPR;
    __shared__ acc4 red[HEAD_MAX_OUT][256];
    __shared__ ACC redb[HEAD_MAX_OUT][256];
    const int sub = threadIdx.x % LPR, rloc = threadIdx.x / LPR;
    f32x4 wv[HEAD_MAX_OUT];
    acc4 dwv[HEAD_MAX_OUT];
    ACC dbv[HEAD_MAX_OUT];
#pragma unroll
    for (int o = 0; o < HEAD_MAX_OUT; ++o) {
        wv[o] = o < Cout ? ldv(w + o * Cin + 4 * sub) : f32x4{0.f, 0.f, 0.f, 0.f};
        dwv[o] = acc4{0, 0, 0, 0};
        dbv[o] = 0;
    }
    const int r0 = blockIdx.x * rows_per_block, r1 = min(M, r0 + rows_per_block);
    for (int r = r0 + rloc; r < r1; r += RPB) {
        const f32x4 xv = ldv(x + (size_t)r * Cin + 4 * sub);
        const acc4 xa = HeadAcc<ACC>::of(xv);
        f32x4 dxa = {0.f, 0.f, 0.f, 0.f};
#pragma unroll
        for (int o = 0; o < HEAD_MAX_OUT; ++o) {
            if (o < Cout) {
                const ACC yy = y[(size_t)r * Cout + o];
                const ACC ga = (ACC)dy[(size_t)r * Cout + o] * ((ACC)1 - yy * yy);
                const float g = (float)ga;
                dxa += g * wv[o];
                dwv[o] += ga * xa;
                dbv[o] += ga;
            }
        }
        if (dx) stv(dx + (size_t)r * Cin + 4 * sub, dxa);
    }
#pragma unroll
    for (int o = 0; o < HEAD_MAX_OUT; ++o) { red[o][threadIdx.x] = dwv[o]; redb[o][threadIdx.x] = dbv[o]; }
    __syncthreads();
    if (rloc == 0) {
        for (int o = 0; o < Cout; ++o) {
            acc4 t = red[o][sub];
            for (int q = 1; q < RPB; ++q) t += red[o][q * LPR + sub];
            *reinterpret_cast<acc4*>(partial + ((size_t)blockIdx.x * HEAD_MAX_OUT + o) * (Cin + 4) + 4 * sub) = t;
            if (sub == 0) {
                ACC tb = 0;
                for (int q = 0; q < RPB; ++q) tb += redb[o][q * LPR];
                partial[((size_t)blockIdx.x * HEAD_MAX_OUT + o) * (Cin + 4) + Cin] = tb;
            }
        }
    }
}

template <typename ACC>
__global__ __launch_bounds__(256) void k_head_reduce(const ACC* __restrict__ partial, int chunks, int Cin, int Cout,
                                                      float* __restrict__ dw, float* __restrict__ db) {
    const int lane = threadIdx.x & 63;
    const int i = blockIdx.x * 4 + (threadIdx.x >> 6);
    if (i >= Cout * (Cin + 1)) return;
    const int o = i / (Cin + 1), c = i % (Cin + 1);
    double s = 0.0;
    for (int k = lane; k < chunks; k += 64) s += partial[((size_t)k * HEAD_MAX_OUT + o) * (Cin + 4) + c];
#pragma unroll
    for (int d = 32; d >= 1; d >>= 1) s += __shfl_xor(s, d, 64);
    if (lane == 0) {
        if (c < Cin) dw[o * Cin + c] = (float)s;
        else db[o] = (float)s;
    }
}

bool head_supported(int Cin, int Cout) {
    return Cout >= 1 && Cout <= HEAD_MAX_OUT && (Cin == 16 || Cin == 32 || Cin == 64 || Cin == 128 || Cin == 256);
}
int head_chunks(int M) { return std::min(1024, (M + 63) / 64); }
bool head_sums_in_double(int M) { return M < HEAD_F64_ROWS; }

#define ICN_HEAD_DISPATCH(KERNEL, ...)                                                  \
    switch (Cin) {                                                                      \
        case 16: hipLaunchKernelGGL((KERNEL<4>), __VA_ARGS__); break;                   \
        case 32: hipLaunchKernelGGL((KERNEL<8>), __VA_ARGS__); break;                   \
        case 64: hipLaunchKernelGGL((KERNEL<16>), __VA_ARGS__); break;                  \
        case 128: hipLaunchKernelGGL((KERNEL<32>), __VA_ARGS__); break;                 \
        default: hipLaunchKernelGGL((KERNEL<64>), __VA_ARGS__); break;                  \
    }

void launch_head_fwd(const float* x, const float* w, const float* bias, float* y, int M, int Cin, int Cout, hipStream_t s) {
    const int rpb = 256 / (Cin / 4);
    const int blocks = std::min(4096, (M + rpb - 1) / rpb);
    ICN_HEAD_DISPATCH(k_head_fwd, dim3(blocks), dim3(256), 0, s, x, w, bias, y, M, Cout)
}

template <typename ACC>
static void head_bwd(const float* dy, const float* y, const float* x, const float* w, float* dx, float* dw, float* db, ACC* ws, int M,
                     int Cin, int Cout, hipStream_t s) {
    const int chunks = head_chunks(M), rows = (M + chunks - 1) / chunks;
    const dim3 grid(chunks), block(256);
    switch (Cin) {
        case 16: hipLaunchKernelGGL((k_head_bwd<4, ACC>), grid, block, 0, s, dy, y, x, w, dx, ws, M, Cout, rows); break;
        case 32: hipLaunchKernelGGL((k_head_bwd<8, ACC>), grid, block, 0, s, dy, y, x, w, dx, ws, M, Cout, rows); break;
        case 64: hipLaunchKernelGGL((k_head_bwd<16, ACC>), grid, block, 0, s, dy, y, x, w, dx, ws, M, Cout, rows); break;
        case 128: hipLaunchKernelGGL((k_head_bwd<32, ACC>), grid, block, 0, s, dy, y, x, w, dx, ws, M, Cout, rows); break;
        default: hipLaunchKernelGGL((k_head_bwd<64, ACC>), grid, block, 0, s, dy, y, x, w, dx, ws, M, Cout, rows); break;
    }
    hipLaunchKernelGGL(k_head_reduce<ACC>, dim3((Cout * (Cin + 1) + 3) / 4), block, 0, s, ws, chunks, Cin, Cout, dw, db);
}

void launch_head_bwd(const float* dy, const float* y, const float* x, const float* w, float* dx, float* dw, float* db, float* ws,
                     int M, int Cin, int Cout, hipStream_t s) {
    if (head_sums_in_double(M)) head_bwd<double>(dy, y, x, w, dx, dw, db, reinterpret_cast<double*>(ws), M, Cin, Cout, s);
    else head_bwd<float>(dy, y, x, w, dx, dw, db, ws, M, Cin, Cout, s);
}
#undef ICN_HEAD_DISPATCH

}
```

geniconet_amd/csrc/icn_launch.h:

```cpp
#pragma once
#include <hip/hip_runtime.h>
#include <stdint.h>

namespace icn {

constexpr int MAX_SEGS = 5;
struct RowSegs {
    int nseg;
    int B;
    int row0[MAX_SEGS], cnt[MAX_SEGS], off[MAX_SEGS];
    unsigned mask[MAX_SEGS];
};

struct GatherGemmArgs {
    const float* src;
    const float* src2;
    const float* wt;
    const float* bias;
    float* dst;
    float* dst2;
    int N0;
    const int32_t* idx;
    const int32_t* dcode;
    const float* side;
    const float* side2;
    int n_slots;
    const int32_t* perm;
    const uint32_t* mask32;
    const uint32_t* mask32_host;
    int mask_key;
    int M, Ps, Pd, K, N, E, ns;
    double algo_flops;
    int T;
    RowSegs segs;
    float* sk_part;
    int* sk_flag;
    int arith_bn;
};
int arith_mode();
int set_arith_mode(int mode);
unsigned build_flags();
int conv_b3_bn(const GatherGemmArgs& a);
constexpr int CONV_SK_ERROR = 1024;
constexpr int CONV_SK_FLAGS = 1032;
void set_trace_buffer(void* p, size_t n_u64);
int* device_status_word();
int device_status(int clear);
size_t conv_sk_part_bytes();
const int* sk_speed_factors(int occ);
}
#include <vector>
namespace icn {
void build_tile_lists(const uint32_t* mask32_host, int M, int Pd, int bm, int ntn, int ntiles, int grid, int occ, std::vector<int>& h);


struct WgradArgs {
    const float* x;
    const float* dy;
    const float* dy2;
    int Cout0;
    const int32_t* idx;
    const int32_t* dcode;
    const float* side;
    int n_slots;
    float* partial;
    float* bias_partial;
    float* dw;
    float* dbias;
    float* dw2;
    float* dbias2;
    int M, Ps, Pd, Cin, Cout, ns;
    double algo_flops;
    int y_taps;
    int identity_rows;
    const int32_t* w7_rows;
    const uint16_t* w7_pos;
    int w7_U;
};

bool gather_gemm_supported(int K, int N);
bool conv_dma_usable(const GatherGemmArgs& a);
void launch_gather_gemm_auto(const GatherGemmArgs& a, hipStream_t s);

bool wgrad_supported(int Cin, int Cout);
bool wgrad_pair_supported(int M, int Ps, int Pd, int Cin, int Cout0, int Cout1);
int wgrad_splits(int M, int Cin, int Cout, int Cout0 = 0);
int wgrad7_splits(int M, int Pd, int Cin, int Cout, int Cout0);
void launch_wgrad(const WgradArgs& a, hipStream_t s);
bool stem_supported(int Cin, int Cout);
void launch_stem_fwd(const float* x, const float* w, const float* bias, float* y, const int32_t* idx, int M, int Ps, int Pd,
                     int Cin, int Cout, int ns, hipStream_t s);

void launch_upconv_gather(const float* dy0, const float* dy1, float* g, const int32_t* idx, const float* coef, const int32_t* rows,
                          int B, int Pin, int nrows, int rows_total, int C0, int C1, int W, int acc, hipStream_t s);

struct PatchTab { const int32_t* prow; const uint16_t* plocal; int npatch, umax, gridW; };
bool upconv_patch_usable(const PatchTab& t, int B, size_t rows_per_sample, int C0, int C1);
void launch_upconv_scatter_lds(const float* z, const float* bias, float* y0, float* y1, const PatchTab& t, const float* coef, int B,
                               int zrows, int Pout, int C0, int C1, hipStream_t s);
void launch_upconv_gather_lds(const float* dy0, const float* dy1, float* g, const PatchTab& t, const int32_t* cls,
                              const float* cls_coef, int ncls, int B, int Pin, int Pc, int C0, int C1, hipStream_t s);

constexpr int UPCONV_PX_CLASSES = 32;
void launch_upconv_gather_px(const float* dy0, const float* dy1, float* g, const int32_t* srcs, const int32_t* cls,
                             const float* cls_coef, int ncls, int B, int Pin, int Pc, int C0, int C1, hipStream_t s);

void launch_upconv_scatter(const float* z, const float* bias, float* y0, float* y1, const int32_t* idx, const float* coef,
                           const int32_t* rows, int B, int zrows, int nrows, int Pout, int C0, int C1, int W, int acc, hipStream_t s);

void launch_spmm_ell(const float* in, float* out, const int32_t* idx, const float* coef, int B, int Pin, int Pout, int C,
                     int W, hipStream_t s);

void launch_conv_generic(const float* src, const float* w, const float* bias, float* dst, const int32_t* idx, int B, int Ps,
                         int Pd, int K, int N, int E, int ns, int transpose, hipStream_t s);

void launch_row_scatter_add(const float* src, float* dst, const int32_t* q, int B, int nv, int nvp, int P, int C, hipStream_t s);

struct PrologueArgs {
    const float* w; const float* w2; float* packed; int Cout, Cout2, Cin, transpose;
    const float* bias; const float* bias2; float* bias_cat;
    const float* src; const float* src2; const int32_t* slots; float* side; float* side2; int n_slots, E, B, Ps, K, ns;
    int* zero; int n_zero;
    int b3_flat_n;
    void* packed_b3; int b3_bn;
};
void launch_conv_prologue(const PrologueArgs& a, hipStream_t s);

struct UpconvPrologueArgs {
    const float* w; const float* w2; float* packed; int Cout, Cout2, Cin, NV; const float* alpha;
    const float* bias; const float* bias2; float* bias_cat;
    const float* src; const int32_t* slot_idx; const float* slot_coef; float* side; int n_slots, E, B, Ps;
};
void launch_upconv_prologue(const UpconvPrologueArgs& a, hipStream_t s);

bool bn_supported(int C);
int bn_chunks(int M);
void launch_bn_stats(const float* x, int M, int C, float eps, float momentum, float* running_mean, float* running_var, float* stat,
                     float* ws, hipStream_t s);
void launch_bn_stats2(const float* a, const float* b, int M, int C, float eps_a, float mom_a, float* rm_a, float* rv_a, float* stat_a,
                      float eps_b, float mom_b, float* rm_b, float* rv_b, float* stat_b, float* ws, hipStream_t s);
void launch_bn_relu_fwd(const float* a, const float* b, const float* stat_a, const float* stat_b, const float* ga, const float* ba,
                        const float* gb, const float* bb, float* y, int M, int C, hipStream_t s);
void launch_bn_relu_bwd(const float* dy, const float* a, const float* b, const float* stat_a, const float* stat_b, const float* ga,
                        const float* ba, const float* gb, const float* bb, float* da, float* db, float* sums, float* ws, int M, int C,
                        float* dbeta_a, float* dgamma_a, float* dbeta_b, float* dgamma_b, hipStream_t s);

bool head_supported(int Cin, int Cout);
int head_chunks(int M);
bool head_sums_in_double(int M);
void launch_head_fwd(const float* x, const float* w, const float* bias, float* y, int M, int Cin, int Cout, hipStream_t s);
void launch_head_bwd(const float* dy, const float* y, const float* x, const float* w, float* dx, float* dw, float* db, float* ws,
                     int M, int Cin, int Cout, hipStream_t s);

int p2p_loss_blocks(int B, int P);
void launch_p2p_loss_fwd(const float* grid, const float* target, const int32_t* vf, float* partial, float* terms, int B, int P, int n,
                         float f_pos, float f_nor, float f_lap, int lap_mode, hipStream_t s);
void launch_p2p_loss_bwd_pos(const float* grid, const float* target, const float* upstream, float f_pos, float* dgrid, int B, int P,
                             int n, hipStream_t s);
void launch_p2p_loss_bwd(const float* grid, const float* target, const int32_t* vf, const float* upstream, float f_pos, float f_nor,
                         float f_lap, int lap_mode, float* dgrid, float* aux, int B, int P, int n, hipStream_t s);
void launch_mesh_reg_fwd(const float* grid, const int32_t* vs, float* partial, float* terms, int B, int P, int n, float f_edge,
                         float f_ncons, float f_smooth, float edge_length, hipStream_t s);
void launch_mesh_reg_bwd(const float* grid, const int32_t* vs, const float* upstream, float f_edge, float f_ncons, float f_smooth,
                         float edge_length, float* dgrid, float* aux, int B, int P, int n, hipStream_t s);

int kld_blocks(size_t n);
void launch_kld_fwd(const float* mu, const float* logvar, size_t n, float* out, float* partial, hipStream_t s);
void launch_kld_bwd(const float* mu, const float* logvar, const float* upstream, size_t n, float* dmu, float* dlogvar, hipStream_t s);
void launch_reparam_fwd(const float* mu, const float* logvar, const float* eps, size_t n, float* z, hipStream_t s);
void launch_reparam_bwd(const float* dz, const float* logvar, const float* eps, size_t n, float* dmu, float* dlogvar, hipStream_t s);

void launch_point_to_mesh(const float* pts, const float* vts, const int32_t* faces, int B, int P, int V, int F, float* dist,
                          int32_t* face, int32_t* kind, hipStream_t s);
void launch_point_to_mesh_bwd(const float* pts, const float* vts, const int32_t* faces, const int32_t* face, const int32_t* kind,
                              const float* ddist, int B, int P, int V, int F, float* dpts, float* dvts, void* ws, hipStream_t s);

int p2m_grid_res(int F);
size_t point_to_mesh_grid_bytes(int B, int F);
hipError_t launch_point_to_mesh_grid(const float* pts, const float* vts, const int32_t* faces, int B, int P, int V, int F, float* dist,
                                     int32_t* face, int32_t* kind, void* ws, hipStream_t s);

size_t mesh_sample_cdf_bytes(int B, int F);
void launch_mesh_sample_fwd(const float* vts, const int32_t* faces, const float* u, int B, int S, int V, int F, float* points,
                            int32_t* face, float* weights, void* ws, hipStream_t s);
void launch_mesh_sample_bwd(const int32_t* faces, const int32_t* face, const float* weights, const float* dpoints, int B, int S, int V,
                            int F, float* dvts, void* ws, hipStream_t s);

size_t vertex_records_bytes(size_t n);
void launch_vertex_scatter(int prof_kind, void* ws, int B, int n, int V, float* dvts, hipStream_t s);

void launch_face_normal_agree_fwd(const float* va, const int32_t* faces_a, const int32_t* face_a, int Va, int Fa, const float* vb,
                                  const int32_t* faces_b, const int32_t* face_b, int Vb, int Fb, int B, int S, int oriented, float* t,
                                  hipStream_t s);
void launch_face_normal_agree_bwd(const float* va, const int32_t* faces_a, const int32_t* face_a, int Va, int Fa, const float* vb,
                                  const int32_t* faces_b, const int32_t* face_b, int Vb, int Fb, int B, int S, int oriented,
                                  const float* dt, float* dva, float* dvb, void* ws, hipStream_t s);

size_t mesh_measure_bytes(int B, int F);
void launch_mesh_measure_fwd(const float* vts, const int32_t* faces, int B, int V, int F, float* area, float* volume, void* ws,
                             hipStream_t s);
void launch_mesh_measure_bwd(const float* vts, const int32_t* faces, const int32_t* offsets, const int32_t* corners, const float* darea,
                             const float* dvolume, int B, int V, int F, float* dvts, hipStream_t s);

size_t mesh_willmore_bytes(int B, int V);
void launch_mesh_cotlap_fwd(const float* vts, const int32_t* faces, const int32_t* offsets, const int32_t* corners, int B, int V, int F,
                            float* lap, float* varea, hipStream_t s);
void launch_mesh_cotlap_bwd(const float* vts, const int32_t* faces, const int32_t* offsets, const int32_t* corners, const float* dlap,
                            const float* dvarea, int B, int V, int F, float* dvts, hipStream_t s);
void launch_mesh_willmore_fwd(const float* vts, const int32_t* faces, const int32_t* offsets, const int32_t* corners, int B, int V, int F,
                              float* lap, float* varea, float* energy, void* ws, hipStream_t s);
void launch_mesh_willmore_bwd(const float* vts, const int32_t* faces, const int32_t* offsets, const int32_t* corners, const float* lap,
                              const float* varea, const float* denergy, int B, int V, int F, float* dvts, void* ws, hipStream_t s);

void launch_mesh_angle_defect_fwd(const float* vts, const int32_t* faces, const int32_t* offsets, const int32_t* corners, int B, int V,
                                  int F, float* defect, hipStream_t s);
void launch_mesh_angle_defect_bwd(const float* vts, const int32_t* faces, const int32_t* offsets, const int32_t* corners,
                                  const float* ddefect, int B, int V, int F, float* dvts, hipStream_t s);

void launch_mesh_self_intersect(const float* vts, const int32_t* faces, int B, int V, int F, int32_t* hits, hipStream_t s);

void launch_point_to_mesh_sign(const float* pts, const float* vts, const int32_t* faces, const int32_t* adjacency, const int32_t* offsets,
                               const int32_t* corners, const int32_t* face, const int32_t* kind, int B, int P, int V, int F, float* sign,
                               hipStream_t s);

constexpr int VOXEL_MAX_DEPTH = 512;
void launch_mesh_voxelize(const float* vts, const int32_t* faces, int B, int V, int F, double ox, double oy, double oz, double h, int n0,
                          int n1, int n2, uint8_t* occ, hipStream_t s);

void launch_mesh_raycast(const float* org, const float* dir, const float* vts, const int32_t* faces, int B, int R, int V, int F, float* depth,
                         int32_t* face, int32_t* count, hipStream_t s);
void launch_mesh_raycast_bwd(const float* org, const float* dir, const float* vts, const int32_t* faces, const int32_t* face,
                             const float* ddepth, int B, int R, int V, int F, float* dorg, float* ddir, float* dvts, void* ws, hipStream_t s);

void launch_nearest_points(const float* pts, const float* tgt, int B, int N, int M, float* dist, int32_t* idx, hipStream_t s);
void launch_nearest_points_bwd(const float* pts, const float* tgt, const int32_t* idx, const float* ddist, int B, int N, int M,
                               float* dpts, float* dtgt, void* ws, hipStream_t s);

size_t sided_sums_workspace_bytes(int G, int R, int N);
void launch_sided_sums(const float* qry, const float* tgt, int G, int R, int N, int M, double* sums, void* ws, hipStream_t s);

bool match_clouds_fits(int N);
size_t match_clouds_workspace_bytes(int G, int R, int N, int paired);
void launch_match_clouds(const float* qry, const float* tgt, int G, int R, int N, int paired, int phases, int max_rounds, int* match,
                         double* prices, double* cost, int* rounds, void* ws, hipStream_t s);

int debug_flags();
int set_debug_flags(int flags);

enum ProfKind { PROF_DMA_128x128 = 0, PROF_DMA_128x64, PROF_DMA_64x128, PROF_DMA_64x64, PROF_GG_128x128, PROF_GG_128x64,
                PROF_GG_64x128, PROF_GG_64x64, PROF_WGD_128x128, PROF_WGD_128x64, PROF_WGD_64x128, PROF_WGD_64x64, PROF_WG_128x128,
                PROF_WG_128x64, PROF_WG_64x128, PROF_WG_64x64,
                PROF_DMAS_128x128, PROF_DMAS_128x64, PROF_DMAS_64x128, PROF_DMAS_64x64,
                PROF_DMAK_64x128, PROF_DMAK_64x64, PROF_DMAKS_64x128, PROF_DMAKS_64x64,
                PROF_WG7,
                PROF_DMA8_64x128, PROF_DMAS8_64x128, PROF_DMAK8_64x128, PROF_DMAKS8_64x128,
                PROF_DENSEK_64x128, PROF_DENSEK_64x64,
                PROF_SINGLEK_64x128, PROF_SINGLEK_64x64,
                PROF_WGDENSE_128x128, PROF_WGDENSE_128x64, PROF_WGDENSE_64x128, PROF_WGDENSE_64x64,
                PROF_B3K_128x128, PROF_B3K_128x64, PROF_B3DENSEK_128x128, PROF_B3DENSEK_128x64,
                PROF_WG7_B3, PROF_WGD_B3, PROF_WGDENSE_B3, PROF_B3_MASKED, PROF_B3SINGLEK_128x128, PROF_B3SINGLEK_128x64,
                PROF_P2M, PROF_P2M_BWD_POINT, PROF_P2M_BWD_VERTEX,
                PROF_P2M_GRID_BOUNDS, PROF_P2M_GRID_COUNT, PROF_P2M_GRID_SCAN, PROF_P2M_GRID_FILL, PROF_P2M_GRID_QUERY,
                PROF_MSAMPLE_AREA, PROF_MSAMPLE_SCAN, PROF_MSAMPLE_POINT, PROF_MSAMPLE_BWD_RECORD, PROF_MSAMPLE_BWD_VERTEX,
                PROF_FNORMAL_AGREE, PROF_FNORMAL_AGREE_BWD_RECORD, PROF_FNORMAL_AGREE_BWD_VERTEX,
                PROF_MESH_MEASURE_FACE, PROF_MESH_MEASURE_FINISH, PROF_MESH_MEASURE_BWD,
                PROF_MESH_COTLAP_FWD, PROF_MESH_WILLMORE_FINISH, PROF_MESH_WILLMORE_UPSTREAM, PROF_MESH_COTLAP_BWD,
                PROF_MESH_ANGLE_DEFECT_FWD, PROF_MESH_ANGLE_DEFECT_BWD,
                PROF_MESH_SELF_INTERSECT,
                PROF_P2M_SIGN,
                PROF_MESH_VOXELIZE,
                PROF_MESH_RAYCAST, PROF_MESH_RAYCAST_BWD_RECORD, PROF_MESH_RAYCAST_BWD_VERTEX,
                PROF_NN, PROF_NN_BWD_RECORD, PROF_NN_BWD_VERTEX,
                PROF_PAIR_SUMS, PROF_PAIR_SUMS_FINISH,
                PROF_MATCH_AUCTION,
                PROF_KINDS };
extern const char* const PROF_NAMES[PROF_KINDS];
void prof_mark_begin(int kind, double flops, hipStream_t s);
void prof_mark_end(hipStream_t s);

constexpr int ADAM_MAX_TENSORS = 96;
void launch_adam(int count, float* const* p, const float* const* g, float* const* m, float* const* v, const size_t* numel,
                 const float* step_size, const float* bc2_sqrt, double beta1, double beta2, double eps, double weight_decay, hipStream_t s,
                 const float* scal_dev = nullptr);

}
```

geniconet_amd/fused.py:

```python
import os
import weakref

import torch

from . import _gradbuf, _lib
from .ico_conv import (_nhwc, ico_conv_pair, ico_conv_pair_supported, ico_upconv_pair,
                       ico_upconv_pair_supported)

_DISABLED = os.environ.get('ICN_NO_FUSED_BN', '') == '1'


def _bn_shape_ok(bn):
    if not (bn.affine and bn.track_running_stats):
        return False
    if bn._forward_hooks or bn._forward_pre_hooks or bn._backward_hooks:
        return False
    c = bn.num_features
    return not (c % 4 or c > 1024 or 256 % (c // 4))


def can_fuse(x, *bns):
    if _DISABLED or not x.is_cuda or x.dtype != torch.float32:
        return False
    return all(bn.training and bn.momentum is not None and _bn_shape_ok(bn) for bn in bns)


def can_fuse_eval(x, *bns):
    if _DISABLED or not x.is_cuda or x.dtype != torch.float32:
        return False
    if torch.is_grad_enabled() and (x.requires_grad or any(bn.weight.requires_grad or bn.bias.requires_grad for bn in bns)):
        return False
    return all((not bn.training) and _bn_shape_ok(bn) for bn in bns)


_NO_PAIR = os.environ.get('ICN_NO_PAIR', '') == '1'


def conv_pair(x, conv_a, conv_b):
    ok = (not _NO_PAIR and x.is_cuda and x.dtype == torch.float32
          and conv_a.stride == conv_b.stride and conv_a.subdivisions == conv_b.subdivisions
          and conv_a.corner_mode == conv_b.corner_mode and (conv_a.bias is None) == (conv_b.bias is None))
    if ok:
        for m in (conv_a, conv_b):
            if m._forward_hooks or m._forward_pre_hooks or m._backward_hooks:
                ok = False
    if ok and ico_conv_pair_supported(x, conv_a.weight, conv_b.weight, conv_a.subdivisions, conv_a.stride):
        return ico_conv_pair(x, conv_a.weight, conv_a.bias, conv_b.weight, conv_b.bias, conv_a.subdivisions,
                             conv_a.stride, conv_a.corner_mode)
    return conv_a(x), conv_b(x)


_NO_UPCONV = os.environ.get('ICN_NO_UPCONV', '') == '1'


def upconv_pair(x, up_a, up_b, conv_a, conv_b):
    mods = (up_a, up_b, conv_a, conv_b)
    plain = not any(m._forward_hooks or m._forward_pre_hooks or m._backward_hooks for m in mods)
    same = (up_a.subdivisions == up_b.subdivisions and up_a.corner_mode == up_b.corner_mode == conv_a.corner_mode
            == conv_b.corner_mode and conv_a.stride == conv_b.stride == 1
            and conv_a.subdivisions == conv_b.subdivisions == up_a.subdivisions + 1
            and (conv_a.bias is None) == (conv_b.bias is None))
    if plain and same and not _NO_PAIR and not _NO_UPCONV and x.is_cuda and x.dtype == torch.float32 \
            and ico_upconv_pair_supported(x, conv_a.weight, conv_b.weight, up_a.subdivisions):
        return ico_upconv_pair(x, conv_a.weight, conv_a.bias, conv_b.weight, conv_b.bias, up_a.subdivisions, up_a.corner_mode)
    up = up_a(x)
    hooked = up_b._forward_hooks or up_b._forward_pre_hooks
    up_skip = up_b(x) if hooked else up
    if up_skip is up:
        return conv_pair(up, conv_a, conv_b)
    return conv_a(up), conv_b(up_skip)


class _BnReluFn(torch.autograd.Function):

    @staticmethod
    def forward(ctx, a, ga, ba, rm_a, rv_a, eps_a, mom_a, b, gb, bb, rm_b, rv_b, eps_b, mom_b):
        L = _lib.api()
        ap = _nhwc(a)
        Bn, H, W, C = ap.shape
        M = Bn * H * W
        dual = b is not None
        bp = _nhwc(b) if dual else None
        dev = a.device
        ws = _lib.workspace(L.icn_bn_workspace_floats(M, C), dev, torch.float32)
        stat_a = torch.empty(2 * C, dtype=torch.float32, device=dev)
        stat_b = torch.empty(2 * C, dtype=torch.float32, device=dev) if dual else None
        y = torch.empty_like(ap)
        with torch.cuda.device(dev):
            st = _lib.stream()
            if dual:
                L.icn_bn_stats2(ap.data_ptr(), bp.data_ptr(), M, C, eps_a, mom_a, rm_a.data_ptr(), rv_a.data_ptr(),
                                stat_a.data_ptr(), eps_b, mom_b, rm_b.data_ptr(), rv_b.data_ptr(), stat_b.data_ptr(),
                                ws.data_ptr(), st)
            else:
                L.icn_bn_stats(ap.data_ptr(), M, C, eps_a, mom_a, rm_a.data_ptr(), rv_a.data_ptr(), stat_a.data_ptr(),
                               ws.data_ptr(), st)
            L.icn_bn_relu_fwd(ap.data_ptr(), bp.data_ptr() if dual else None, stat_a.data_ptr(),
                              stat_b.data_ptr() if dual else None, ga.data_ptr(), ba.data_ptr(),
                              gb.data_ptr() if dual else None, bb.data_ptr() if dual else None, y.data_ptr(), M, C, st)
        ctx.save_for_backward(ap, bp, stat_a, stat_b, ga, ba, gb, bb)
        ctx.dims = (M, C, dual)
        ctx.params = (ga, ba, gb, bb)
        return y.permute(0, 3, 1, 2)

    @staticmethod
    @torch.autograd.function.once_differentiable
    def backward(ctx, gy):
        L = _lib.api()
        ap, bp, stat_a, stat_b, ga, ba, gb, bb = ctx.saved_tensors
        M, C, dual = ctx.dims
        gyp = _nhwc(gy)
        dev = gyp.device
        da = torch.empty_like(ap)
        db = torch.empty_like(bp) if dual else None
        sums = torch.empty(3 * C, dtype=torch.float32, device=dev)
        ws = _lib.workspace(L.icn_bn_workspace_floats(M, C), dev, torch.float32)
        pga, pba, pgb, pbb = ctx.params
        dga, dba = _gradbuf.lease(pga, (C,), dev), _gradbuf.lease(pba, (C,), dev)
        dgb = _gradbuf.lease(pgb, (C,), dev) if dual else None
        dbb = _gradbuf.lease(pbb, (C,), dev) if dual else None
        with torch.cuda.device(dev):
            L.icn_bn_relu_bwd(gyp.data_ptr(), ap.data_ptr(), bp.data_ptr() if dual else None, stat_a.data_ptr(),
                              stat_b.data_ptr() if dual else None, ga.data_ptr(), ba.data_ptr(),
                              gb.data_ptr() if dual else None, bb.data_ptr() if dual else None, da.data_ptr(),
                              db.data_ptr() if dual else None, sums.data_ptr(), ws.data_ptr(), M, C, dba.data_ptr(),
                              dga.data_ptr(), dbb.data_ptr() if dual else None, dgb.data_ptr() if dual else None, _lib.stream())
        out = [da.permute(0, 3, 1, 2), dga, dba, None, None, None, None]
        if dual:
            out += [db.permute(0, 3, 1, 2), dgb, dbb, None, None, None, None]
        else:
            out += [None] * 7
        return tuple(out)


def _args(bn):
    return bn.weight, bn.bias, bn.running_mean, bn.running_var, float(bn.eps), float(bn.momentum)


_pending_counters = []
_defer_depth = 0


class counters_deferred:
    def __enter__(self):
        global _defer_depth
        _defer_depth += 1

    def __exit__(self, *exc):
        global _defer_depth
        _defer_depth -= 1
        if _defer_depth == 0 and _pending_counters:
            todo = list(_pending_counters)
            _pending_counters.clear()
            torch._foreach_add_(todo, 1)
        return False


def _bump(bn):
    _eval_stats.pop(bn, None)
    if _defer_depth > 0:
        _pending_counters.append(bn.num_batches_tracked)
    else:
        bn.num_batches_tracked.add_(1)


def bn_relu(a, bn):
    _bump(bn)
    return _BnReluFn.apply(a, *_args(bn), None, None, None, None, None, 0.0, 0.0)


def bn_add_relu(a, bn_a, b, bn_b):
    _bump(bn_a)
    _bump(bn_b)
    return _BnReluFn.apply(a, *_args(bn_a), b, *_args(bn_b))


_eval_stats = weakref.WeakKeyDictionary()


def _eval_stat(bn):
    rm, rv = bn.running_mean, bn.running_var
    key = (rm._version, rv._version, rm.data_ptr(), rv.data_ptr(), float(bn.eps))
    hit = _eval_stats.get(bn)
    if hit is None or hit[0] != key:
        hit = (key, torch.cat([rm.detach().float(), torch.rsqrt(rv.detach().float() + bn.eps)]))
        _eval_stats[bn] = hit
    return hit[1]


def _bn_relu_eval(a, bn_a, b=None, bn_b=None):
    L = _lib.api()
    ap = _nhwc(a.detach())
    Bn, H, W, C = ap.shape
    M = Bn * H * W
    dual = b is not None
    bp = _nhwc(b.detach()) if dual else None
    stat_a = _eval_stat(bn_a)
    stat_b = _eval_stat(bn_b) if dual else None
    y = torch.empty_like(ap)
    with torch.cuda.device(a.device):
        L.icn_bn_relu_fwd(ap.data_ptr(), bp.data_ptr() if dual else None, stat_a.data_ptr(),
                          stat_b.data_ptr() if dual else None, bn_a.weight.data_ptr(), bn_a.bias.data_ptr(),
                          bn_b.weight.data_ptr() if dual else None, bn_b.bias.data_ptr() if dual else None,
                          y.data_ptr(), M, C, _lib.stream())
    return y.permute(0, 3, 1, 2)


def bn_relu_eval(a, bn):
    return _bn_relu_eval(a, bn)


def bn_add_relu_eval(a, bn_a, b, bn_b):
    return _bn_relu_eval(a, bn_a, b, bn_b)


class _HeadFn(torch.autograd.Function):

    @staticmethod
    def forward(ctx, x, weight, bias):
        L = _lib.api()
        xp = _nhwc(x)
        Bn, H, W, Cin = xp.shape
        Cout, M = weight.shape[0], Bn * H * W
        w2 = weight.reshape(Cout, Cin).contiguous()
        y = torch.empty(Bn, H, W, Cout, dtype=torch.float32, device=x.device)
        with torch.cuda.device(x.device):
            L.icn_head_fwd(xp.data_ptr(), w2.data_ptr(), bias.contiguous().data_ptr(), y.data_ptr(), M, Cin, Cout, _lib.stream())
        ctx.save_for_backward(xp, w2, y)
        ctx.wshape, ctx.wstride = weight.shape, weight.stride()
        ctx.params = (weight, bias)
        return y.permute(0, 3, 1, 2)

    @staticmethod
    @torch.autograd.function.once_differentiable
    def backward(ctx, gy):
        L = _lib.api()
        xp, w2, y = ctx.saved_tensors
        Bn, H, W, Cin = xp.shape
        Cout, M = w2.shape[0], Bn * H * W
        gyp = _nhwc(gy)
        dev = gyp.device
        dx = torch.empty_like(xp) if ctx.needs_input_grad[0] else None
        dw = _gradbuf.lease(ctx.params[0], ctx.wshape, dev, stride=ctx.wstride)
        db = _gradbuf.lease(ctx.params[1], (Cout,), dev)
        ws = _lib.workspace(L.icn_head_workspace_floats(M, Cin), dev, torch.float32)
        with torch.cuda.device(dev):
            L.icn_head_bwd(gyp.data_ptr(), y.data_ptr(), xp.data_ptr(), w2.data_ptr(),
                           dx.data_ptr() if dx is not None else None, dw.data_ptr(), db.data_ptr(), ws.data_ptr(), M,
                           Cin, Cout, _lib.stream())
        return (dx.permute(0, 3, 1, 2) if dx is not None else None), dw, db


def can_fuse_head(x, seq):
    if _DISABLED or not x.is_cuda or x.dtype != torch.float32 or len(seq) != 2:
        return False
    conv, act = seq[0], seq[1]
    if not isinstance(conv, torch.nn.Conv2d) or not isinstance(act, torch.nn.Tanh):
        return False
    if conv.kernel_size != (1, 1) or conv.stride != (1, 1) or conv.padding != (0, 0) or conv.groups != 1 or conv.bias is None:
        return False
    if conv.in_channels not in (16, 32, 64, 128, 256) or conv.out_channels > 4:
        return False
    for m in (seq, conv, act):
        if m._forward_hooks or m._forward_pre_hooks or m._backward_hooks:
            return False
    return True


def head(x, seq):
    if can_fuse_head(x, seq):
        return _HeadFn.apply(x, seq[0].weight, seq[0].bias)
    return seq(x)


class _ReparamFn(torch.autograd.Function):

    @staticmethod
    def forward(ctx, mu, logvar, eps):
        L = _lib.api()
        m, lv, e = _nhwc(mu), _nhwc(logvar), _nhwc(eps)
        z = torch.empty_like(m)
        with torch.cuda.device(m.device):
            L.icn_reparam_fwd(m.data_ptr(), lv.data_ptr(), e.data_ptr(), m.numel(), z.data_ptr(), _lib.stream())
        ctx.save_for_backward(lv, e)
        return z.permute(0, 3, 1, 2)

    @staticmethod
    @torch.autograd.function.once_differentiable
    def backward(ctx, gz):
        L = _lib.api()
        lv, e = ctx.saved_tensors
        g = _nhwc(gz)
        dm, dlv = torch.empty_like(g), torch.empty_like(g)
        with torch.cuda.device(g.device):
            L.icn_reparam_bwd(g.data_ptr(), lv.data_ptr(), e.data_ptr(), g.numel(), dm.data_ptr(), dlv.data_ptr(), _lib.stream())
        return dm.permute(0, 3, 1, 2), dlv.permute(0, 3, 1, 2), None


def reparameterize(mu, logvar):
    if (not _DISABLED and mu.is_cuda and logvar.is_cuda and mu.dtype == torch.float32 and logvar.dtype == torch.float32
            and mu.dim() == 4 and mu.shape == logvar.shape and mu.numel() > 0):
        return _ReparamFn.apply(mu, logvar, torch.randn_like(logvar))
    std = torch.exp(0.5 * logvar)
    return torch.randn_like(std) * std + mu
```

geniconet_amd/models.py:

```python
import torch
from torch import nn
from torch.nn import functional as F

from . import fused
from .ico_conv import IcoConvS2S, IcoUpsampleS2S

STEM_CHANNELS = 64
DOWN_CHANNELS = (128, 256, 256)
UP_CHANNELS = (256, 128, 64)
VAE_LATENT_CHANNELS = 512


class BasicIcoS2SDownBlock(nn.Module):

    def __init__(self, in_features, out_features, bias, in_subdivisions, corner_mode):
        super().__init__()
        kw = dict(bias=bias, corner_mode=corner_mode)
        self.conv00 = IcoConvS2S(in_features, out_features, stride=2, subdivisions=in_subdivisions, **kw)
        self.icobn00 = nn.BatchNorm2d(out_features)
        self.conv01 = IcoConvS2S(out_features, out_features, stride=1, subdivisions=in_subdivisions - 1, **kw)
        self.icobn01 = nn.BatchNorm2d(out_features)
        self.conv10 = IcoConvS2S(in_features, out_features, stride=2, subdivisions=in_subdivisions, **kw)
        self.icobn10 = nn.BatchNorm2d(out_features)

    def forward(self, x):
        c00, c10 = fused.conv_pair(x, self.conv00, self.conv10)
        if fused.can_fuse(x, self.icobn00, self.icobn01, self.icobn10):
            h = fused.bn_relu(c00, self.icobn00)
            return fused.bn_add_relu(self.conv01(h), self.icobn01, c10, self.icobn10)
        if fused.can_fuse_eval(x, self.icobn00, self.icobn01, self.icobn10):
            h = fused.bn_relu_eval(c00, self.icobn00)
            return fused.bn_add_relu_eval(self.conv01(h), self.icobn01, c10, self.icobn10)
        main = self.icobn01(self.conv01(F.relu(self.icobn00(c00))))
        skip = self.icobn10(c10)
        return F.relu(main + skip)


class BasicIcoS2SUpBlock(nn.Module):

    def __init__(self, in_features, out_features, bias, in_subdivisions, corner_mode):
        super().__init__()
        kw = dict(stride=1, bias=bias, subdivisions=in_subdivisions + 1, corner_mode=corner_mode)
        self.upsample00 = IcoUpsampleS2S(in_features, in_subdivisions, corner_mode)
        self.conv00 = IcoConvS2S(in_features, out_features, **kw)
        self.icobn00 = nn.BatchNorm2d(out_features)
        self.conv01 = IcoConvS2S(out_features, out_features, **kw)
        self.icobn01 = nn.BatchNorm2d(out_features)
        self.upsample10 = IcoUpsampleS2S(in_features, in_subdivisions, corner_mode)
        self.conv10 = IcoConvS2S(in_features, out_features, **kw)
        self.icobn10 = nn.BatchNorm2d(out_features)

    def forward(self, x):
        c00, c10 = fused.upconv_pair(x, self.upsample00, self.upsample10, self.conv00, self.conv10)
        if fused.can_fuse(x, self.icobn00, self.icobn01, self.icobn10):
            h = fused.bn_relu(c00, self.icobn00)
            return fused.bn_add_relu(self.conv01(h), self.icobn01, c10, self.icobn10)
        if fused.can_fuse_eval(x, self.icobn00, self.icobn01, self.icobn10):
            h = fused.bn_relu_eval(c00, self.icobn00)
            return fused.bn_add_relu_eval(self.conv01(h), self.icobn01, c10, self.icobn10)
        main = self.icobn01(self.conv01(F.relu(self.icobn00(c00))))
        skip = self.icobn10(c10)
        return F.relu(main + skip)


class IcoUpS2S(nn.Module):

    def __init__(self, in_features, out_features, bias=True, subdivisions=0, corner_mode='zeros'):
        super().__init__()
        self.up = IcoUpsampleS2S(in_features, subdivisions, corner_mode)
        self.conv = IcoConvS2S(in_features, out_features, 1, bias, subdivisions + 1, corner_mode=corner_mode)

    def forward(self, x):
        return self.conv(self.up(x))


def _check_model(model):
    if model != 'residualS2S':
        raise ValueError("only model='residualS2S' is built (reference models.py:102,135); got %r" % (model,))


class _Encoder(nn.Sequential):

    def forward(self, x):
        mods = list(self)
        x = mods[0](x)
        relu = mods[2]
        hooked = relu._forward_hooks or relu._forward_pre_hooks or relu._backward_hooks
        if isinstance(relu, nn.ReLU) and not hooked and fused.can_fuse(x, mods[1]):
            x = fused.bn_relu(x, mods[1])
        elif isinstance(relu, nn.ReLU) and not hooked and isinstance(mods[1], nn.BatchNorm2d) and fused.can_fuse_eval(x, mods[1]):
            x = fused.bn_relu_eval(x, mods[1])
        else:
            x = relu(mods[1](x))
        for m in mods[3:]:
            x = m(x)
        return x


def _encoder(corner_mode, subdivisions, n_down):
    layers = [IcoConvS2S(3, STEM_CHANNELS, 1, True, subdivisions, corner_mode),
              nn.BatchNorm2d(STEM_CHANNELS), nn.ReLU(inplace=False)]
    cin = STEM_CHANNELS
    for k in range(n_down):
        layers.append(BasicIcoS2SDownBlock(cin, DOWN_CHANNELS[k], True, subdivisions - k, corner_mode))
        cin = DOWN_CHANNELS[k]
    return _Encoder(*layers)


def _decoder(corner_mode, subdivisions, latent_channels):
    blocks, cin = [], latent_channels
    for k, cout in enumerate(UP_CHANNELS):
        blocks.append(BasicIcoS2SUpBlock(cin, cout, True, subdivisions - 3 + k, corner_mode))
        cin = cout
    head = nn.Sequential(nn.Conv2d(cin, 3, kernel_size=(1, 1)), nn.Tanh())
    return nn.Sequential(*blocks), head


def createico2enc(corner_mode='average', model='simple', subdivisions=5):
    _check_model(model)
    return _encoder(corner_mode, subdivisions, 3)


def createenc2ico(corner_mode='average', model='simple', subdivisions=5):
    _check_model(model)
    return _decoder(corner_mode, subdivisions, DOWN_CHANNELS[-1])


def createico2enc_vae(corner_mode='average', model='simple', subdivisions=5):
    _check_model(model)
    return _encoder(corner_mode, subdivisions, 2)


def createenc2ico_vae(corner_mode='average', model='simple', subdivisions=5):
    _check_model(model)
    return _decoder(corner_mode, subdivisions, VAE_LATENT_CHANNELS)


def _levels(params):
    return params['ico'].get('subdivisions', 5)


class ico2ico(nn.Module):

    def __init__(self, params):
        super().__init__()
        mode, kind, R = params['ico']['corner_mode'], params['ico2ico']['model'], _levels(params)
        self.encoder = createico2enc(mode, kind, R)
        self.enc = nn.Identity()
        self.subdivisions = R
        self.decoder, self.enc2icoConv = createenc2ico(mode, kind, R)

    def forward(self, x):
        with fused.counters_deferred():
            return fused.head(self.decoder(self.enc(self.encoder(x))), self.enc2icoConv)


class ico2enc(nn.Module):

    def __init__(self, params):
        super().__init__()
        self.encoder = createico2enc(params['ico']['corner_mode'], params['ico2ico']['model'], _levels(params))

    def forward(self, x):
        return self.encoder(x)


class enc2ico(nn.Module):

    def __init__(self, params):
        super().__init__()
        self.subdivisions = _levels(params)
        self.decoder, self.enc2icoConv = createenc2ico(params['ico']['corner_mode'], params['ico2ico']['model'],
                                                       self.subdivisions)

    def forward(self, x):
        return fused.head(self.decoder(x), self.enc2icoConv)


class VAE(nn.Module):

    def __init__(self):
        super().__init__()
        self.encoder = self.mu = self.logvar = self.decoder = None

    def encode(self, input):
        raise NotImplementedError

    def decode(self, input):
        raise NotImplementedError

    def reparameterize(self, mu, logvar):
        return fused.reparameterize(mu, logvar)

    def forward(self, x):
        with fused.counters_deferred():
            mu, logvar = self.encode(x)
            return self.decode(self.reparameterize(mu, logvar)), mu, logvar


def _latent_head(corner_mode, subdivisions):
    return nn.Sequential(IcoConvS2S(DOWN_CHANNELS[1], VAE_LATENT_CHANNELS, 2, True, subdivisions - 2, corner_mode),
                         nn.BatchNorm2d(VAE_LATENT_CHANNELS))


def _latent_heads(mu, logvar, h):
    plain = all(isinstance(m, nn.Sequential) and len(m) == 2 and isinstance(m[0], IcoConvS2S)
                and not (m._forward_hooks or m._forward_pre_hooks or m._backward_hooks) for m in (mu, logvar))
    if not plain:
        return mu(h), logvar(h)
    a, b = fused.conv_pair(h, mu[0], logvar[0])
    return mu[1](a), logvar[1](b)


class ico2ico_vae(VAE):

    def __init__(self, params):
        super().__init__()
        self.params = params
        self.model = params[params['model_name']]['model']
        mode, R = params['ico']['corner_mode'], _levels(params)
        self.encoder = createico2enc_vae(mode, self.model, R)
        self.mu = self.createMu()
        self.logvar = self.createLogvar()
        self.mu_hook = nn.Identity()
        self.logvar_hook = nn.Identity()
        self.reparameterize_hook = nn.Identity()
        self.subdivisions = R
        self.decoder, self.final_layer = createenc2ico_vae(mode, self.model, R)

    def createMu(self):
        return _latent_head(self.params['ico']['corner_mode'], _levels(self.params))

    def createLogvar(self):
        return _latent_head(self.params['ico']['corner_mode'], _levels(self.params))

    def encode(self, input):
        m, lv = _latent_heads(self.mu, self.logvar, self.encoder(input))
        return self.mu_hook(m), self.logvar_hook(lv)

    def decode(self, z):
        return fused.head(self.decoder(self.reparameterize_hook(z)), self.final_layer)


class ico2enc_vae(VAE):

    def __init__(self, params):
        super().__init__()
        self.params = params
        self.model = params[params['model_name']]['model']
        self.encoder = createico2enc_vae(params['ico']['corner_mode'], self.model, _levels(params))
        self.mu = ico2ico_vae.createMu(self)
        self.logvar = ico2ico_vae.createLogvar(self)

    def encode(self, input):
        return _latent_heads(self.mu, self.logvar, self.encoder(input))

    def forward(self, x):
        return self.encode(x)


class enc2ico_vae(VAE):

    def __init__(self, params):
        super().__init__()
        self.params = params
        self.model = params[params['model_name']]['model']
        self.subdivisions = _levels(params)
        self.decoder, self.final_layer = createenc2ico_vae(params['ico']['corner_mode'], self.model, self.subdivisions)

    def createSample(self, batch_size, misc):
        mean, logvar = misc[0]['trn_mean'], misc[0]['trn_logvar']
        return torch.add(mean, logvar * torch.randn(logvar.shape))

    def decode(self, z):
        return fused.head(self.decoder(z), self.final_layer)

    def forward(self, x):
        return self.decode(x), torch.tensor([]), torch.tensor([])


def default_params(model_name='ico2ico', subdivisions=5, corner_mode='average'):
    p = {'model_name': model_name,
         'ico': {'corner_mode': corner_mode, 'subdivisions': subdivisions, 'width': 2 ** (subdivisions + 1)},
         'ico2ico': {'model': 'residualS2S', 'loss': 'p2p', 'lr': 1e-6, 'lr_base': 1e-9, 'lr_max': 1e-3},
         'ico2ico_vae': {'model': 'residualS2S', 'loss': 'p2pkld', 'lr': 1e-6, 'lr_base': 1e-9, 'lr_max': 1e-3,
                         'factor_step_size': 25, 'factor_gamma': 0.9}}
    if model_name == 'ico2ico':
        p['ico'].update(factor_pos=1., factor_nor=0., factor_lap=0.)
    else:
        p['ico'].update(factor_pos=0.6, factor_nor=0.2, factor_lap=0.2)
    return p
```

Before: 5705 meshes/s.

## Fuse final decoder block's BN-add-ReLU with tanh head conv

Adds fused HIP kernels that apply the last up-block's dual batchnorm, residual add and ReLU, then the 1x1 tanh output head, in one pass. The backward pass gets matching kernels that compute head gradients, BN gradient sums and input gradients without ever storing the activated tensor. This is meant to remove a full-resolution write and re-read of the largest activation plus several kernel launches at the I5 level. In exchange it adds new code paths with an env-var opt-out and more complex backward reductions.

```diff
diff --git a/geniconet_amd/_lib.py b/geniconet_amd/_lib.py
--- a/geniconet_amd/_lib.py
+++ b/geniconet_amd/_lib.py
@@ -156,6 +156,13 @@
                              + [ctypes.c_void_p, ctypes.c_size_t, ctypes.c_void_p], RC),
     },
 }
+FUSED_HEADERS = {
+    'icn_fused.h': {
+        'icn_bn_head_workspace_bytes': (ctypes.c_size_t, [ctypes.c_int] * 3, PLAIN),
+        'icn_bn_head_fwd': (ctypes.c_int, [_c_float_p] * 11 + [ctypes.c_int] * 3 + [ctypes.c_void_p], RC),
+        'icn_bn_head_bwd': (ctypes.c_int, [_c_float_p] * 20 + [ctypes.c_int] * 3 + [ctypes.c_void_p, ctypes.c_size_t, ctypes.c_void_p], RC),
+    },
+}
 
 
 class ProfileEntry(ctypes.Structure):
@@ -188,7 +195,7 @@
                 '(or `make -C geniconet_amd/csrc`).' % LIB_PATH)
         handle = ctypes.CDLL(LIB_PATH)
         checked = types.SimpleNamespace()
-        for name, (res, args, reply) in [item for table in (SIGNATURES, *EXTENSION_HEADERS.values(), *LATER_HEADERS.values(), *MATCH_HEADERS.values()) for item in table.items()]:
+        for name, (res, args, reply) in [item for table in (SIGNATURES, *EXTENSION_HEADERS.values(), *LATER_HEADERS.values(), *MATCH_HEADERS.values(), *FUSED_HEADERS.values()) for item in table.items()]:
             fn = getattr(handle, name)
             fn.restype, fn.argtypes = res, args
             fn = handle[name]
@@ -243,7 +250,7 @@
 
 def source_files():
     import glob
-    headers = [os.path.join(os.path.dirname(_HERE), 'include', h) for h in ('icn.h', *EXTENSION_HEADERS, *LATER_HEADERS, *MATCH_HEADERS)]
+    headers = [os.path.join(os.path.dirname(_HERE), 'include', h) for h in ('icn.h', *EXTENSION_HEADERS, *LATER_HEADERS, *MATCH_HEADERS, *FUSED_HEADERS)]
     return sorted([f for pattern in ('*.hip', '*.h', '*.cpp') for f in glob.glob(os.path.join(_HERE, 'csrc', pattern))] + headers)
 
 
diff --git a/geniconet_amd/csrc/icn_api.cpp b/geniconet_amd/csrc/icn_api.cpp
--- a/geniconet_amd/csrc/icn_api.cpp
+++ b/geniconet_amd/csrc/icn_api.cpp
@@ -22,6 +22,7 @@
 #include "../../include/icn_nn.h"
 #include "../../include/icn_pairs.h"
 #include "../../include/icn_match.h"
+#include "../../include/icn_fused.h"
 #include "../../include/icn_measure.h"
 #include "icn_geometry.h"
 #include "icn_launch.h"
@@ -1823,6 +1824,42 @@
     });
 }
 
+namespace {
+bool bn_head_sizes_ok(int M, int C, int Cout) { return M >= 1 && icn::bn_supported(C) && icn::head_supported(C, Cout); }
+}
+
+size_t icn_bn_head_workspace_bytes(int M, int C, int Cout) {
+    return bn_head_sizes_ok(M, C, Cout) ? icn::bn_head_workspace_bytes(M, C) : 0;
+}
+
+int icn_bn_head_fwd(const float* a, const float* b, const float* stat_a, const float* stat_b, const float* gamma_a, const float* beta_a,
+                    const float* gamma_b, const float* beta_b, const float* w, const float* bias, float* y, int M, int C, int Cout,
+                    void* stream) {
+    hipStream_t s = static_cast<hipStream_t>(stream);
+    return launched([&] {
+        if (!a || !b || !stat_a || !stat_b || !gamma_a || !beta_a || !gamma_b || !beta_b || !w || !bias || !y)
+            throw std::invalid_argument("icn_bn_head_fwd: null pointer");
+        if (!bn_head_sizes_ok(M, C, Cout)) throw std::invalid_argument("icn_bn_head_fwd: bad sizes");
+        icn::launch_bn_head_fwd(a, b, stat_a, stat_b, gamma_a, beta_a, gamma_b, beta_b, w, bias, y, M, C, Cout, s);
+    });
+}
+
+int icn_bn_head_bwd(const float* dy, const float* y, const float* a, const float* b, const float* stat_a, const float* stat_b,
+                    const float* gamma_a, const float* beta_a, const float* gamma_b, const float* beta_b, const float* w, float* da,
+                    float* db, float* sums, float* dw, float* dbias, float* dbeta_a, float* dgamma_a, float* dbeta_b, float* dgamma_b,
+                    int M, int C, int Cout, void* ws, size_t ws_bytes, void* stream) {
+    hipStream_t s = static_cast<hipStream_t>(stream);
+    return launched([&] {
+        if (!dy || !y || !a || !b || !stat_a || !stat_b || !gamma_a || !beta_a || !gamma_b || !beta_b || !w || !da || !db || !sums || !dw ||
+            !dbias)
+            throw std::invalid_argument("icn_bn_head_bwd: null pointer");
+        if (!bn_head_sizes_ok(M, C, Cout)) throw std::invalid_argument("icn_bn_head_bwd: bad sizes");
+        check_workspace("icn_bn_head_bwd", ws, ws_bytes, icn::bn_head_workspace_bytes(M, C));
+        icn::launch_bn_head_bwd(dy, y, a, b, stat_a, stat_b, gamma_a, beta_a, gamma_b, beta_b, w, da, db, sums, dw, dbias, dbeta_a,
+                                dgamma_a, dbeta_b, dgamma_b, ws, M, C, Cout, s);
+    });
+}
+
 long icn_table_conv_fwd(int r_in, int stride, int corner_mode, int32_t* out, size_t cap) {
     return returns<long>([&] {
         std::vector<int32_t> v;
diff --git a/geniconet_amd/csrc/icn_bn.hip b/geniconet_amd/csrc/icn_bn.hip
--- a/geniconet_amd/csrc/icn_bn.hip
+++ b/geniconet_amd/csrc/icn_bn.hip
@@ -3,6 +3,7 @@
 
 #include <algorithm>
 
+#include "icn_bn_device.h"
 #include "icn_launch.h"
 
 #ifndef ICN_CHAIN_PRIO
@@ -16,27 +17,11 @@
 
 namespace icn {
 
-using f32x4 = __attribute__((ext_vector_type(4))) float;
-__device__ __forceinline__ f32x4 ldv(const float* p) { return *reinterpret_cast<const f32x4*>(p); }
-__device__ __forceinline__ void stv(float* p, f32x4 v) { *reinterpret_cast<f32x4*>(p) = v; }
-__device__ __forceinline__ f32x4 relu4(f32x4 v) { return f32x4{fmaxf(v[0], 0.f), fmaxf(v[1], 0.f), fmaxf(v[2], 0.f), fmaxf(v[3], 0.f)}; }
-
 #ifndef ICN_BN_MAX_CHUNKS
 #define ICN_BN_MAX_CHUNKS 512
 #endif
 constexpr int BN_MAX_CHUNKS = ICN_BN_MAX_CHUNKS;
 static_assert(BN_MAX_CHUNKS >= 1 && BN_MAX_CHUNKS <= 65536, "ICN_BN_MAX_CHUNKS");
-
-using f64x4 = __attribute__((ext_vector_type(4))) double;
-__device__ __forceinline__ f64x4 to_d(f32x4 v) { return f64x4{(double)v[0], (double)v[1], (double)v[2], (double)v[3]}; }
-
-template <int DUAL>
-__device__ __forceinline__ f32x4 bn_pre4(f32x4 a, f32x4 mean_a, f32x4 scale_a, f32x4 beta_a, f32x4 b, f32x4 mean_b, f32x4 scale_b,
-                                         f32x4 beta_b) {
-    f32x4 v = (a - mean_a) * scale_a + beta_a;
-    if (DUAL) v += (b - mean_b) * scale_b + beta_b;
-    return v;
-}
 
 #ifndef ICN_BN_UN
 #define ICN_BN_UN 4
@@ -338,6 +323,12 @@
     else hipLaunchKernelGGL(k_bn_relu_fwd<0>, dim3(stream_blocks(total4)), dim3(256), 0, s, a, b, stat_a, stat_b, ga, ba, gb, bb, y, total4, C);
 }
 
+void launch_bn_finalize_bwd(const double* partial, int chunks, int C, int NS, float* sums, float* dbeta_a, float* dgamma_a,
+                            float* dbeta_b, float* dgamma_b, hipStream_t s) {
+    hipLaunchKernelGGL(k_bn_finalize_bwd, dim3((C + 15) / 16, NS), dim3(256), 0, s, partial, chunks, C, NS, sums,
+                       BnGradOut{dbeta_a, dbeta_b, dgamma_a, dgamma_b});
+}
+
 void launch_bn_relu_bwd(const float* dy, const float* a, const float* b, const float* stat_a, const float* stat_b, const float* ga,
                         const float* ba, const float* gb, const float* bb, float* da, float* db, float* sums, float* ws, int M, int C,
                         float* dbeta_a, float* dgamma_a, float* dbeta_b, float* dgamma_b, hipStream_t s) {
@@ -346,8 +337,7 @@
     double* wsd = reinterpret_cast<double*>(ws);
     if (b) hipLaunchKernelGGL(k_bn_partial<2>, dim3(chunks), dim3(256), 0, s, dy, a, b, stat_a, stat_b, ga, ba, gb, bb, wsd, M, C, rows);
     else hipLaunchKernelGGL(k_bn_partial<1>, dim3(chunks), dim3(256), 0, s, dy, a, b, stat_a, stat_b, ga, ba, gb, bb, wsd, M, C, rows);
-    hipLaunchKernelGGL(k_bn_finalize_bwd, dim3((C + 15) / 16, NS), dim3(256), 0, s, wsd, chunks, C, NS, sums,
-                       BnGradOut{dbeta_a, b ? dbeta_b : nullptr, dgamma_a, b ? dgamma_b : nullptr});
+    launch_bn_finalize_bwd(wsd, chunks, C, NS, sums, dbeta_a, dgamma_a, b ? dbeta_b : nullptr, b ? dgamma_b : nullptr, s);
     const size_t total4 = (size_t)M * C / 4;
     if (b) hipLaunchKernelGGL(k_bn_relu_bwd<1>, dim3(stream_blocks(total4)), dim3(256), 0, s, dy, a, b, stat_a, stat_b, ga, ba, gb, bb, sums, da, db, total4, C, 1.f / M);
     else hipLaunchKernelGGL(k_bn_relu_bwd<0>, dim3(stream_blocks(total4)), dim3(256), 0, s, dy, a, b, stat_a, stat_b, ga, ba, gb, bb, sums, da, db, total4, C, 1.f / M);
@@ -356,8 +346,6 @@
 }
 
 namespace icn {
-
-constexpr int HEAD_MAX_OUT = 4;
 
 template <int LPR>
 __global__ __launch_bounds__(256) void k_head_fwd(const float* __restrict__ x, const float* __restrict__ w,
@@ -386,9 +374,6 @@
 }
 
 constexpr int HEAD_F64_ROWS = 1024;
-template <typename ACC> struct HeadAcc;
-template <> struct HeadAcc<float> { using v4 = f32x4; static __device__ __forceinline__ v4 of(f32x4 v) { return v; } };
-template <> struct HeadAcc<double> { using v4 = f64x4; static __device__ __forceinline__ v4 of(f32x4 v) { return to_d(v); } };
 
 template <int LPR, typename ACC>
 __global__ __launch_bounds__(256) void k_head_bwd(const float* __restrict__ dy, const float* __restrict__ y,
@@ -497,6 +482,12 @@
     hipLaunchKernelGGL(k_head_reduce<ACC>, dim3((Cout * (Cin + 1) + 3) / 4), block, 0, s, ws, chunks, Cin, Cout, dw, db);
 }
 
+void launch_head_reduce(const void* partial, bool in_double, int chunks, int Cin, int Cout, float* dw, float* db, hipStream_t s) {
+    const dim3 grid((Cout * (Cin + 1) + 3) / 4), block(256);
+    if (in_double) hipLaunchKernelGGL(k_head_reduce<double>, grid, block, 0, s, static_cast<const double*>(partial), chunks, Cin, Cout, dw, db);
+    else hipLaunchKernelGGL(k_head_reduce<float>, grid, block, 0, s, static_cast<const float*>(partial), chunks, Cin, Cout, dw, db);
+}
+
 void launch_head_bwd(const float* dy, const float* y, const float* x, const float* w, float* dx, float* dw, float* db, float* ws,
                      int M, int Cin, int Cout, hipStream_t s) {
     if (head_sums_in_double(M)) head_bwd<double>(dy, y, x, w, dx, dw, db, reinterpret_cast<double*>(ws), M, Cin, Cout, s);
diff --git a/geniconet_amd/csrc/icn_bn_device.h b/geniconet_amd/csrc/icn_bn_device.h
--- /dev/null
+++ b/geniconet_amd/csrc/icn_bn_device.h
@@ -0,0 +1,67 @@
+#pragma once
+#include <hip/hip_runtime.h>
+
+namespace icn {
+
+using f32x4 = __attribute__((ext_vector_type(4))) float;
+__device__ __forceinline__ f32x4 ldv(const float* p) { return *reinterpret_cast<const f32x4*>(p); }
+__device__ __forceinline__ void stv(float* p, f32x4 v) { *reinterpret_cast<f32x4*>(p) = v; }
+__device__ __forceinline__ f32x4 relu4(f32x4 v) { return f32x4{fmaxf(v[0], 0.f), fmaxf(v[1], 0.f), fmaxf(v[2], 0.f), fmaxf(v[3], 0.f)}; }
+
+using f64x4 = __attribute__((ext_vector_type(4))) double;
+__device__ __forceinline__ f64x4 to_d(f32x4 v) { return f64x4{(double)v[0], (double)v[1], (double)v[2], (double)v[3]}; }
+
+template <int DUAL>
+__device__ __forceinline__ f32x4 bn_pre4(f32x4 a, f32x4 mean_a, f32x4 scale_a, f32x4 beta_a, f32x4 b, f32x4 mean_b, f32x4 scale_b,
+                                         f32x4 beta_b) {
+    f32x4 v = (a - mean_a) * scale_a + beta_a;
+    if (DUAL) v += (b - mean_b) * scale_b + beta_b;
+    return v;
+}
+
+__device__ __forceinline__ f32x4 relu_mask4(f32x4 v, f32x4 dy) {
+    f32x4 g;
+#pragma unroll
+    for (int j = 0; j < 4; ++j) g[j] = v[j] > 0.f ? dy[j] : 0.f;
+    return g;
+}
+
+__device__ __forceinline__ f32x4 bn_dx4(f32x4 g, f32x4 x, f32x4 mean, f32x4 inv, f32x4 gamma, f32x4 sum_g, f32x4 sum_gx, float inv_m) {
+    const f32x4 xh = (x - mean) * inv, scale = gamma * inv;
+    f32x4 d;
+#pragma unroll
+    for (int j = 0; j < 4; ++j) d[j] = scale[j] * __builtin_fmaf(-xh[j], sum_gx[j] * inv_m, __builtin_fmaf(-sum_g[j], inv_m, g[j]));
+    return d;
+}
+
+template <typename ACC> struct HeadAcc;
+template <> struct HeadAcc<float> { using v4 = f32x4; static __device__ __forceinline__ v4 of(f32x4 v) { return v; } };
+template <> struct HeadAcc<double> { using v4 = f64x4; static __device__ __forceinline__ v4 of(f32x4 v) { return to_d(v); } };
+
+__device__ __forceinline__ float fma_acc(float a, float b, float c) { return __builtin_fmaf(a, b, c); }
+__device__ __forceinline__ double fma_acc(double a, double b, double c) { return __builtin_fma(a, b, c); }
+
+template <typename ACC> struct HeadG3 { ACC dy, f, g3; };
+template <typename ACC>
+__device__ __forceinline__ HeadG3<ACC> head_g3(float dy, float y) {
+    HeadG3<ACC> t;
+    const ACC yy = y;
+    t.dy = dy;
+    t.f = fma_acc(-yy, yy, (ACC)1);
+    t.g3 = t.dy * t.f;
+    return t;
+}
+template <typename ACC>
+__device__ __forceinline__ ACC head_dbias_add(ACC sum, const HeadG3<ACC>& t) { return fma_acc(t.dy, t.f, sum); }
+
+constexpr int HEAD_MAX_OUT = 4;
+
+__device__ __forceinline__ f32x4 head_dx4(const float* g3, const f32x4* wv, int Cout) {
+    f32x4 dx = {0.f, 0.f, 0.f, 0.f};
+#pragma unroll
+    for (int o = 0; o < HEAD_MAX_OUT; ++o)
+        if (o < Cout) dx += g3[o] * wv[o];
+    return dx;
+}
+
+}
diff --git a/geniconet_amd/csrc/icn_fused.hip b/geniconet_amd/csrc/icn_fused.hip
--- /dev/null
+++ b/geniconet_amd/csrc/icn_fused.hip
@@ -0,0 +1,280 @@
+#include <hip/hip_runtime.h>
+#include <stdint.h>
+
+#include <algorithm>
+
+#include "icn_bn_device.h"
+#include "icn_launch.h"
+
+namespace icn {
+
+struct TailBn {
+    f32x4 mean_a, inv_a, gam_a, be_a, mean_b, inv_b, gam_b, be_b;
+    __device__ __forceinline__ TailBn(const float* stat_a, const float* stat_b, const float* ga, const float* ba, const float* gb,
+                                      const float* bb, int C, int c)
+        : mean_a(ldv(stat_a + c)), inv_a(ldv(stat_a + C + c)), gam_a(ldv(ga + c)), be_a(ldv(ba + c)), mean_b(ldv(stat_b + c)),
+          inv_b(ldv(stat_b + C + c)), gam_b(ldv(gb + c)), be_b(ldv(bb + c)) {}
+    __device__ __forceinline__ f32x4 pre(f32x4 a, f32x4 b) const {
+        return bn_pre4<1>(a, mean_a, inv_a * gam_a, be_a, b, mean_b, inv_b * gam_b, be_b);
+    }
+};
+
+constexpr int TAIL_UN_FWD = 4, TAIL_UN_SUMS = 2, TAIL_UN_APPLY = 2;
+
+template <int LPR>
+__global__ __launch_bounds__(256) void k_bn_head_fwd(const float* __restrict__ a, const float* __restrict__ b,
+                                                      const float* __restrict__ stat_a, const float* __restrict__ stat_b,
+                                                      const float* __restrict__ ga, const float* __restrict__ ba,
+                                                      const float* __restrict__ gb, const float* __restrict__ bb,
+                                                      const float* __restrict__ w, const float* __restrict__ bias,
+                                                      float* __restrict__ y, int M, int Cout) {
+    constexpr int C = LPR * 4, RPB = 256 / LPR, UN = TAIL_UN_FWD;
+    const int sub = threadIdx.x % LPR, rloc = threadIdx.x / LPR;
+    const TailBn bn(stat_a, stat_b, ga, ba, gb, bb, C, 4 * sub);
+    f32x4 wv[HEAD_MAX_OUT];
+#pragma unroll
+    for (int o = 0; o < HEAD_MAX_OUT; ++o) wv[o] = o < Cout ? ldv(w + o * C + 4 * sub) : f32x4{0.f, 0.f, 0.f, 0.f};
+    const float bs = sub < Cout ? bias[sub] : 0.f;
+    for (long r = (long)blockIdx.x * (RPB * UN) + rloc; r < M; r += (long)gridDim.x * (RPB * UN)) {
+        f32x4 av[UN], bv[UN];
+#pragma unroll
+        for (int u = 0; u < UN; ++u) {
+            const size_t o = (size_t)min(r + u * RPB, (long)M - 1) * C + 4 * sub;
+            av[u] = ldv(a + o);
+            bv[u] = ldv(b + o);
+        }
+#pragma unroll
+        for (int u = 0; u < UN; ++u) {
+            const f32x4 xv = relu4(bn.pre(av[u], bv[u]));
+            float acc[HEAD_MAX_OUT];
+#pragma unroll
+            for (int o = 0; o < HEAD_MAX_OUT; ++o) acc[o] = xv[0] * wv[o][0] + xv[1] * wv[o][1] + xv[2] * wv[o][2] + xv[3] * wv[o][3];
+#pragma unroll
+            for (int d = LPR / 2; d >= 1; d >>= 1)
+#pragma unroll
+                for (int o = 0; o < HEAD_MAX_OUT; ++o) acc[o] += __shfl_xor(acc[o], d, 64);
+            float v = acc[0];
+#pragma unroll
+            for (int o = 1; o < HEAD_MAX_OUT; ++o) v = sub == o ? acc[o] : v;
+            const long ru = r + u * RPB;
+            if (ru < M && sub < Cout) y[(size_t)ru * Cout + sub] = tanhf(v + bs);
+        }
+    }
+}
+
+template <typename ACC> struct TailRow { f32x4 x, g; HeadG3<ACC> g3[HEAD_MAX_OUT]; };
+template <typename ACC>
+__device__ __forceinline__ TailRow<ACC> tail_row(const TailBn& bn, f32x4 av, f32x4 bv, const float* dyv, const float* yv,
+                                                 const f32x4* wv, int Cout) {
+    TailRow<ACC> t;
+    float g3f[HEAD_MAX_OUT];
+#pragma unroll
+    for (int o = 0; o < HEAD_MAX_OUT; ++o) {
+        t.g3[o] = head_g3<ACC>(dyv[o], yv[o]);
+        g3f[o] = (float)t.g3[o].g3;
+    }
+    const f32x4 v = bn.pre(av, bv);
+    t.x = relu4(v);
+    t.g = relu_mask4(v, head_dx4(g3f, wv, Cout));
+    return t;
+}
+
+template <int LPR, typename ACC>
+__global__ __launch_bounds__(256) void k_bn_head_bwd_sums(const float* __restrict__ dy, const float* __restrict__ y,
+                                                           const float* __restrict__ a, const float* __restrict__ b,
+                                                           const float* __restrict__ stat_a, const float* __restrict__ stat_b,
+                                                           const float* __restrict__ ga, const float* __restrict__ ba,
+                                                           const float* __restrict__ gb, const float* __restrict__ bb,
+                                                           const float* __restrict__ w, double* __restrict__ bn_part,
+                                                           ACC* __restrict__ head_part, int M, int Cout, int rows_per_chunk) {
+    using acc4 = typename HeadAcc<ACC>::v4;
+    constexpr int C = LPR * 4, RPB = 256 / LPR, UN = TAIL_UN_SUMS;
+    __shared__ f64x4 red[256];
+    const int sub = threadIdx.x % LPR, rloc = threadIdx.x / LPR;
+    const TailBn bn(stat_a, stat_b, ga, ba, gb, bb, C, 4 * sub);
+    f32x4 wv[HEAD_MAX_OUT];
+    acc4 dwv[HEAD_MAX_OUT];
+    ACC dbv[HEAD_MAX_OUT];
+#pragma unroll
+    for (int o = 0; o < HEAD_MAX_OUT; ++o) {
+        wv[o] = o < Cout ? ldv(w + o * C + 4 * sub) : f32x4{0.f, 0.f, 0.f, 0.f};
+        dwv[o] = acc4{0, 0, 0, 0};
+        dbv[o] = 0;
+    }
+    f64x4 q[3];
+#pragma unroll
+    for (int k = 0; k < 3; ++k) q[k] = f64x4{0.0, 0.0, 0.0, 0.0};
+    const int r0 = blockIdx.x * rows_per_chunk, r1 = min(M, r0 + rows_per_chunk);
+    for (int r = r0 + rloc; r < r1; r += UN * RPB) {
+        f32x4 av[UN], bv[UN];
+        float dyv[UN][HEAD_MAX_OUT], yv[UN][HEAD_MAX_OUT];
+#pragma unroll
+        for (int u = 0; u < UN; ++u) {
+            const size_t row = (size_t)min(r + u * RPB, r1 - 1);
+            av[u] = ldv(a + row * C + 4 * sub);
+            bv[u] = ldv(b + row * C + 4 * sub);
+#pragma unroll
+            for (int o = 0; o < HEAD_MAX_OUT; ++o) {
+                dyv[u][o] = o < Cout ? dy[row * Cout + o] : 0.f;
+                yv[u][o] = o < Cout ? y[row * Cout + o] : 0.f;
+            }
+        }
+#pragma unroll
+        for (int u = 0; u < UN; ++u) {
+            if (r + u * RPB >= r1) continue;
+            const TailRow<ACC> t = tail_row<ACC>(bn, av[u], bv[u], dyv[u], yv[u], wv, Cout);
+            const acc4 xa = HeadAcc<ACC>::of(t.x);
+#pragma unroll
+            for (int o = 0; o < HEAD_MAX_OUT; ++o) {
+                if (o < Cout) {
+                    dwv[o] += t.g3[o].g3 * xa;
+                    dbv[o] = head_dbias_add(dbv[o], t.g3[o]);
+                }
+            }
+            const f64x4 gd = to_d(t.g);
+            q[0] += gd;
+            q[1] += gd * to_d((av[u] - bn.mean_a) * bn.inv_a);
+            q[2] += gd * to_d((bv[u] - bn.mean_b) * bn.inv_b);
+        }
+    }
+#pragma unroll
+    for (int k = 0; k < 3; ++k) {
+        __syncthreads();
+        red[threadIdx.x] = q[k];
+        __syncthreads();
+        if (rloc == 0) {
+            f64x4 t = red[sub];
+#pragma unroll 4
+            for (int g = 1; g < RPB; ++g) t += red[g * LPR + sub];
+            *reinterpret_cast<f64x4*>(bn_part + ((size_t)blockIdx.x * 3 + k) * C + 4 * sub) = t;
+        }
+    }
+    acc4* redw = reinterpret_cast<acc4*>(red);
+    ACC* redb = reinterpret_cast<ACC*>(red);
+    for (int o = 0; o < Cout; ++o) {
+        __syncthreads();
+        redw[threadIdx.x] = dwv[o];
+        __syncthreads();
+        if (rloc == 0) {
+            acc4 t = redw[sub];
+#pragma unroll 4
+            for (int g = 1; g < RPB; ++g) t += redw[g * LPR + sub];
+            *reinterpret_cast<acc4*>(head_part + ((size_t)blockIdx.x * HEAD_MAX_OUT + o) * (C + 4) + 4 * sub) = t;
+        }
+        __syncthreads();
+        redb[threadIdx.x] = dbv[o];
+        __syncthreads();
+        if (threadIdx.x == 0) {
+            ACC tb = 0;
+            for (int g = 0; g < RPB; ++g) tb += redb[g * LPR];
+            head_part[((size_t)blockIdx.x * HEAD_MAX_OUT + o) * (C + 4) + C] = tb;
+        }
+    }
+}
+
+template <int LPR, typename ACC>
+__global__ __launch_bounds__(256) void k_bn_head_bwd_apply(const float* __restrict__ dy, const float* __restrict__ y,
+                                                            const float* __restrict__ a, const float* __restrict__ b,
+                                                            const float* __restrict__ stat_a, const float* __restrict__ stat_b,
+                                                            const float* __restrict__ ga, const float* __restrict__ ba,
+                                                            const float* __restrict__ gb, const float* __restrict__ bb,
+                                                            const float* __restrict__ w, const float* __restrict__ sums,
+                                                            float* __restrict__ da, float* __restrict__ db, int M, int Cout,
+                                                            float inv_m) {
+    constexpr int C = LPR * 4, RPB = 256 / LPR, UN = TAIL_UN_APPLY;
+    const int sub = threadIdx.x % LPR, rloc = threadIdx.x / LPR;
+    const TailBn bn(stat_a, stat_b, ga, ba, gb, bb, C, 4 * sub);
+    f32x4 wv[HEAD_MAX_OUT];
+#pragma unroll
+    for (int o = 0; o < HEAD_MAX_OUT; ++o) wv[o] = o < Cout ? ldv(w + o * C + 4 * sub) : f32x4{0.f, 0.f, 0.f, 0.f};
+    const f32x4 sg = ldv(sums + 4 * sub), sga = ldv(sums + C + 4 * sub), sgb = ldv(sums + 2 * C + 4 * sub);
+    for (long r = (long)blockIdx.x * (RPB * UN) + rloc; r < M; r += (long)gridDim.x * (RPB * UN)) {
+        f32x4 av[UN], bv[UN];
+        float dyv[UN][HEAD_MAX_OUT], yv[UN][HEAD_MAX_OUT];
+#pragma unroll
+        for (int u = 0; u < UN; ++u) {
+            const size_t row = (size_t)min(r + u * RPB, (long)M - 1);
+            av[u] = ldv(a + row * C + 4 * sub);
+            bv[u] = ldv(b + row * C + 4 * sub);
+#pragma unroll
+            for (int o = 0; o < HEAD_MAX_OUT; ++o) {
+                dyv[u][o] = o < Cout ? dy[row * Cout + o] : 0.f;
+                yv[u][o] = o < Cout ? y[row * Cout + o] : 0.f;
+            }
+        }
+#pragma unroll
+        for (int u = 0; u < UN; ++u) {
+            const long ru = r + u * RPB;
+            if (ru >= M) break;
+            const TailRow<ACC> t = tail_row<ACC>(bn, av[u], bv[u], dyv[u], yv[u], wv, Cout);
+            stv(da + (size_t)ru * C + 4 * sub, bn_dx4(t.g, av[u], bn.mean_a, bn.inv_a, bn.gam_a, sg, sga, inv_m));
+            stv(db + (size_t)ru * C + 4 * sub, bn_dx4(t.g, bv[u], bn.mean_b, bn.inv_b, bn.gam_b, sg, sgb, inv_m));
+        }
+    }
+}
+
+static size_t tail_bn_doubles(int M, int C) { return (size_t)head_chunks(M) * 3 * C; }
+size_t bn_head_workspace_bytes(int M, int C) {
+    return (tail_bn_doubles(M, C) + (size_t)head_chunks(M) * HEAD_MAX_OUT * (C + 4)) * sizeof(double);
+}
+
+#define ICN_TAIL_DISPATCH(KERNEL, ...)                                                  \
+    switch (C) {                                                                        \
+        case 16: hipLaunchKernelGGL((KERNEL<4>), __VA_ARGS__); break;                   \
+        case 32: hipLaunchKernelGGL((KERNEL<8>), __VA_ARGS__); break;                   \
+        case 64: hipLaunchKernelGGL((KERNEL<16>), __VA_ARGS__); break;                  \
+        case 128: hipLaunchKernelGGL((KERNEL<32>), __VA_ARGS__); break;                 \
+        default: hipLaunchKernelGGL((KERNEL<64>), __VA_ARGS__); break;                  \
+    }
+#define ICN_TAIL_DISPATCH_ACC(KERNEL, ACC, ...)                                         \
+    switch (C) {                                                                        \
+        case 16: hipLaunchKernelGGL((KERNEL<4, ACC>), __VA_ARGS__); break;              \
+        case 32: hipLaunchKernelGGL((KERNEL<8, ACC>), __VA_ARGS__); break;              \
+        case 64: hipLaunchKernelGGL((KERNEL<16, ACC>), __VA_ARGS__); break;             \
+        case 128: hipLaunchKernelGGL((KERNEL<32, ACC>), __VA_ARGS__); break;            \
+        default: hipLaunchKernelGGL((KERNEL<64, ACC>), __VA_ARGS__); break;             \
+    }
+
+static int tail_blocks(int M, int C, int un) {
+    const int rows = 256 / (C / 4) * un;
+    return std::min(4096, (M + rows - 1) / rows);
+}
+
+void launch_bn_head_fwd(const float* a, const float* b, const float* stat_a, const float* stat_b, const float* ga, const float* ba,
+                        const float* gb, const float* bb, const float* w, const float* bias, float* y, int M, int C, int Cout,
+                        hipStream_t s) {
+    ICN_TAIL_DISPATCH(k_bn_head_fwd, dim3(tail_blocks(M, C, TAIL_UN_FWD)), dim3(256), 0, s, a, b, stat_a, stat_b, ga, ba, gb, bb, w, bias,
+                      y, M, Cout)
+}
+
+template <typename ACC>
+static void bn_head_bwd(const float* dy, const float* y, const float* a, const float* b, const float* stat_a, const float* stat_b,
+                        const float* ga, const float* ba, const float* gb, const float* bb, const float* w, float* da, float* db,
+                        float* sums, float* dw, float* dbias, float* dbeta_a, float* dgamma_a, float* dbeta_b, float* dgamma_b, void* ws,
+                        int M, int C, int Cout, hipStream_t s) {
+    const int chunks = head_chunks(M), rows = (M + chunks - 1) / chunks;
+    double* bn_part = reinterpret_cast<double*>(ws);
+    ACC* head_part = reinterpret_cast<ACC*>(bn_part + tail_bn_doubles(M, C));
+    ICN_TAIL_DISPATCH_ACC(k_bn_head_bwd_sums, ACC, dim3(chunks), dim3(256), 0, s, dy, y, a, b, stat_a, stat_b, ga, ba, gb, bb, w, bn_part,
+                          head_part, M, Cout, rows)
+    launch_bn_finalize_bwd(bn_part, chunks, C, 3, sums, dbeta_a, dgamma_a, dbeta_b, dgamma_b, s);
+    launch_head_reduce(head_part, sizeof(ACC) == sizeof(double), chunks, C, Cout, dw, dbias, s);
+    ICN_TAIL_DISPATCH_ACC(k_bn_head_bwd_apply, ACC, dim3(tail_blocks(M, C, TAIL_UN_APPLY)), dim3(256), 0, s, dy, y, a, b, stat_a, stat_b,
+                          ga, ba, gb, bb, w, sums, da, db, M, Cout, 1.f / M)
+}
+
+void launch_bn_head_bwd(const float* dy, const float* y, const float* a, const float* b, const float* stat_a, const float* stat_b,
+                        const float* ga, const float* ba, const float* gb, const float* bb, const float* w, float* da, float* db,
+                        float* sums, float* dw, float* dbias, float* dbeta_a, float* dgamma_a, float* dbeta_b, float* dgamma_b, void* ws,
+                        int M, int C, int Cout, hipStream_t s) {
+    if (head_sums_in_double(M))
+        bn_head_bwd<double>(dy, y, a, b, stat_a, stat_b, ga, ba, gb, bb, w, da, db, sums, dw, dbias, dbeta_a, dgamma_a, dbeta_b, dgamma_b,
+                            ws, M, C, Cout, s);
+    else
+        bn_head_bwd<float>(dy, y, a, b, stat_a, stat_b, ga, ba, gb, bb, w, da, db, sums, dw, dbias, dbeta_a, dgamma_a, dbeta_b, dgamma_b,
+                           ws, M, C, Cout, s);
+}
+#undef ICN_TAIL_DISPATCH
+#undef ICN_TAIL_DISPATCH_ACC
+
+}
diff --git a/geniconet_amd/csrc/icn_launch.h b/geniconet_amd/csrc/icn_launch.h
--- a/geniconet_amd/csrc/icn_launch.h
+++ b/geniconet_amd/csrc/icn_launch.h
@@ -151,6 +151,18 @@
 void launch_head_fwd(const float* x, const float* w, const float* bias, float* y, int M, int Cin, int Cout, hipStream_t s);
 void launch_head_bwd(const float* dy, const float* y, const float* x, const float* w, float* dx, float* dw, float* db, float* ws,
                      int M, int Cin, int Cout, hipStream_t s);
+
+size_t bn_head_workspace_bytes(int M, int C);
+void launch_bn_head_fwd(const float* a, const float* b, const float* stat_a, const float* stat_b, const float* ga, const float* ba,
+                        const float* gb, const float* bb, const float* w, const float* bias, float* y, int M, int C, int Cout,
+                        hipStream_t s);
+void launch_bn_head_bwd(const float* dy, const float* y, const float* a, const float* b, const float* stat_a, const float* stat_b,
+                        const float* ga, const float* ba, const float* gb, const float* bb, const float* w, float* da, float* db,
+                        float* sums, float* dw, float* dbias, float* dbeta_a, float* dgamma_a, float* dbeta_b, float* dgamma_b, void* ws,
+                        int M, int C, int Cout, hipStream_t s);
+void launch_bn_finalize_bwd(const double* partial, int chunks, int C, int NS, float* sums, float* dbeta_a, float* dgamma_a,
+                            float* dbeta_b, float* dgamma_b, hipStream_t s);
+void launch_head_reduce(const void* partial, bool in_double, int chunks, int Cin, int Cout, float* dw, float* db, hipStream_t s);
 
 int p2p_loss_blocks(int B, int P);
 void launch_p2p_loss_fwd(const float* grid, const float* target, const int32_t* vf, float* partial, float* terms, int B, int P, int n,
diff --git a/geniconet_amd/fused.py b/geniconet_amd/fused.py
--- a/geniconet_amd/fused.py
+++ b/geniconet_amd/fused.py
@@ -273,6 +273,72 @@
     return seq(x)
 
 
+_NO_TAIL = os.environ.get('ICN_NO_FUSED_TAIL', '') == '1'
+
+
+class _BnHeadFn(torch.autograd.Function):
+
+    @staticmethod
+    def forward(ctx, a, ga, ba, rm_a, rv_a, eps_a, mom_a, b, gb, bb, rm_b, rv_b, eps_b, mom_b, weight, bias):
+        L = _lib.api()
+        ap, bp = _nhwc(a), _nhwc(b)
+        Bn, H, W, C = ap.shape
+        Cout, M = weight.shape[0], Bn * H * W
+        dev = a.device
+        w2 = weight.reshape(Cout, C).contiguous()
+        ws = _lib.workspace(L.icn_bn_workspace_floats(M, C), dev, torch.float32)
+        stat_a = torch.empty(2 * C, dtype=torch.float32, device=dev)
+        stat_b = torch.empty(2 * C, dtype=torch.float32, device=dev)
+        y = torch.empty(Bn, H, W, Cout, dtype=torch.float32, device=dev)
+        with torch.cuda.device(dev):
+            st = _lib.stream()
+            L.icn_bn_stats2(ap.data_ptr(), bp.data_ptr(), M, C, eps_a, mom_a, rm_a.data_ptr(), rv_a.data_ptr(), stat_a.data_ptr(),
+                            eps_b, mom_b, rm_b.data_ptr(), rv_b.data_ptr(), stat_b.data_ptr(), ws.data_ptr(), st)
+            L.icn_bn_head_fwd(ap.data_ptr(), bp.data_ptr(), stat_a.data_ptr(), stat_b.data_ptr(), ga.data_ptr(), ba.data_ptr(),
+                              gb.data_ptr(), bb.data_ptr(), w2.data_ptr(), bias.contiguous().data_ptr(), y.data_ptr(), M, C, Cout, st)
+        ctx.save_for_backward(ap, bp, stat_a, stat_b, ga, ba, gb, bb, w2, y)
+        ctx.wshape, ctx.wstride = weight.shape, weight.stride()
+        ctx.params = (ga, ba, gb, bb, weight, bias)
+        return y.permute(0, 3, 1, 2)
+
+    @staticmethod
+    @torch.autograd.function.once_differentiable
+    def backward(ctx, gy):
+        L = _lib.api()
+        ap, bp, stat_a, stat_b, ga, ba, gb, bb, w2, y = ctx.saved_tensors
+        Bn, H, W, C = ap.shape
+        Cout, M = w2.shape[0], Bn * H * W
+        gyp = _nhwc(gy)
+        dev = gyp.device
+        da, db = torch.empty_like(ap), torch.empty_like(bp)
+        sums = torch.empty(3 * C, dtype=torch.float32, device=dev)
+        need = L.icn_bn_head_workspace_bytes(M, C, Cout)
+        ws = _lib.workspace(need, dev)
+        pga, pba, pgb, pbb, pw, pbias = ctx.params
+        dga, dba = _gradbuf.lease(pga, (C,), dev), _gradbuf.lease(pba, (C,), dev)
+        dgb, dbb = _gradbuf.lease(pgb, (C,), dev), _gradbuf.lease(pbb, (C,), dev)
+        dw = _gradbuf.lease(pw, ctx.wshape, dev, stride=ctx.wstride)
+        dbias = _gradbuf.lease(pbias, (Cout,), dev)
+        with torch.cuda.device(dev):
+            L.icn_bn_head_bwd(gyp.data_ptr(), y.data_ptr(), ap.data_ptr(), bp.data_ptr(), stat_a.data_ptr(), stat_b.data_ptr(),
+                              ga.data_ptr(), ba.data_ptr(), gb.data_ptr(), bb.data_ptr(), w2.data_ptr(), da.data_ptr(), db.data_ptr(),
+                              sums.data_ptr(), dw.data_ptr(), dbias.data_ptr(), dba.data_ptr(), dga.data_ptr(), dbb.data_ptr(),
+                              dgb.data_ptr(), M, C, Cout, ws.data_ptr(), need, _lib.stream())
+        return (da.permute(0, 3, 1, 2), dga, dba, None, None, None, None, db.permute(0, 3, 1, 2), dgb, dbb, None, None, None, None,
+                dw, dbias)
+
+
+def can_fuse_tail(x, bn_a, bn_b, seq):
+    return (not _NO_TAIL and can_fuse(x, bn_a, bn_b) and can_fuse_head(x, seq)
+            and seq[0].in_channels == bn_a.num_features == bn_b.num_features)
+
+
+def bn_add_relu_head(a, bn_a, b, bn_b, seq):
+    _bump(bn_a)
+    _bump(bn_b)
+    return _BnHeadFn.apply(a, *_args(bn_a), b, *_args(bn_b), seq[0].weight, seq[0].bias)
+
+
 class _ReparamFn(torch.autograd.Function):
 
     @staticmethod
diff --git a/geniconet_amd/models.py b/geniconet_amd/models.py
--- a/geniconet_amd/models.py
+++ b/geniconet_amd/models.py
@@ -61,6 +61,22 @@
         main = self.icobn01(self.conv01(F.relu(self.icobn00(c00))))
         skip = self.icobn10(c10)
         return F.relu(main + skip)
+
+    def forward_with_head(self, x, head):
+        c00, c10 = fused.upconv_pair(x, self.upsample00, self.upsample10, self.conv00, self.conv10)
+        h = fused.bn_relu(c00, self.icobn00)
+        return fused.bn_add_relu_head(self.conv01(h), self.icobn01, c10, self.icobn10, head)
+
+
+def _decode(decoder, head, x):
+    last = decoder[-1] if isinstance(decoder, nn.Sequential) and len(decoder) else None
+    if isinstance(last, BasicIcoS2SUpBlock) and not any(m._forward_hooks or m._forward_pre_hooks or m._backward_hooks
+                                                       for m in (decoder, last)) \
+            and fused.can_fuse(x, last.icobn00) and fused.can_fuse_tail(x, last.icobn01, last.icobn10, head):
+        for m in list(decoder)[:-1]:
+            x = m(x)
+        return last.forward_with_head(x, head)
+    return fused.head(decoder(x), head)
 
 
 class IcoUpS2S(nn.Module):
@@ -152,7 +168,7 @@
 
     def forward(self, x):
         with fused.counters_deferred():
-            return fused.head(self.decoder(self.enc(self.encoder(x))), self.enc2icoConv)
+            return _decode(self.decoder, self.enc2icoConv, self.enc(self.encoder(x)))
 
 
 class ico2enc(nn.Module):
@@ -174,7 +190,7 @@
                                                        self.subdivisions)
 
     def forward(self, x):
-        return fused.head(self.decoder(x), self.enc2icoConv)
+        return _decode(self.decoder, self.enc2icoConv, x)
 
 
 class VAE(nn.Module):
@@ -239,7 +255,7 @@
         return self.mu_hook(m), self.logvar_hook(lv)
 
     def decode(self, z):
-        return fused.head(self.decoder(self.reparameterize_hook(z)), self.final_layer)
+        return _decode(self.decoder, self.final_layer, self.reparameterize_hook(z))
 
 
 class ico2enc_vae(VAE):
@@ -273,7 +289,7 @@
         return torch.add(mean, logvar * torch.randn(logvar.shape))
 
     def decode(self, z):
-        return fused.head(self.decoder(z), self.final_layer)
+        return _decode(self.decoder, self.final_layer, z)
 
     def forward(self, x):
         return self.decode(x), torch.tensor([]), torch.tensor([])
diff --git a/include/icn_fused.h b/include/icn_fused.h
--- /dev/null
+++ b/include/icn_fused.h
@@ -0,0 +1,24 @@
+#ifndef ICN_FUSED_H
+#define ICN_FUSED_H
+
+#include "icn.h"
+
+#ifdef __cplusplus
+extern "C" {
+#endif
+
+size_t icn_bn_head_workspace_bytes(int M, int C, int Cout);
+
+int icn_bn_head_fwd(const float* a, const float* b, const float* stat_a, const float* stat_b, const float* gamma_a, const float* beta_a,
+                    const float* gamma_b, const float* beta_b, const float* w, const float* bias, float* y, int M, int C, int Cout,
+                    void* stream);
+
+int icn_bn_head_bwd(const float* dy, const float* y, const float* a, const float* b, const float* stat_a, const float* stat_b,
+                    const float* gamma_a, const float* beta_a, const float* gamma_b, const float* beta_b, const float* w, float* da,
+                    float* db, float* sums, float* dw, float* dbias, float* dbeta_a, float* dgamma_a, float* dbeta_b, float* dgamma_b,
+                    int M, int C, int Cout, void* ws, size_t ws_bytes, void* stream);
+
+#ifdef __cplusplus
+}
+#endif
+#endif
```

Result: faster. 5802 meshes/s (median of 6 runs) (+1.7%).
